# apple/ml-4m

Measured on AMD Instinct MI355X. Metric: multimodal tokens/sec (4M-B train step, whole job), higher is better.
Workload: dtype bf16; 1 GPU; 4M-B mod7 (fm_base_12e_12d_swiglu_nobias, 360.8M params, 8 input / 7 target modalities) masked-modeling train step, 224^2 token grids, 128 input + 128 target tokens/sample, AdamW; model=fm_base_12e_12d_swiglu_nobias, per_gpu_batch=256, global_batch=256, seq_len=256, parallelism=dp1

## Files before the change

include/fourm_hip.h:

```cpp
#ifndef FOURM_HIP_H
#define FOURM_HIP_H
#include <stdint.h>

#ifdef __cplusplus
extern "C" {
#endif

#define FM_ABI_VERSION 11
int fm_abi_version(void);
const char* fm_last_error(void);

enum fm_epilogue {
    FM_EPI_BF16 = 0,
    FM_EPI_GELU = 1,
    FM_EPI_RESIDUAL = 2,
    FM_EPI_SWIGLU = 3,
    FM_EPI_F32 = 4,
    FM_EPI_TANH = 5,
    FM_EPI_SWIGLU_BWD = 6,
    FM_EPI_GELU_BWD = 7,
    FM_EPI_QUICK_GELU = 8,
    FM_EPI_RELU = 9,
    FM_EPI_RELU_BWD = 10
};

typedef struct fm_gemm_group {
    const void* W;
    void* out;
    int32_t N, K, ldw, pad_;
} fm_gemm_group;

typedef struct fm_gemm_nt_args {
    const void* W; const void* W2; const void* X;
    void* out; void* out2; const void* res; const void* bias; const void* bias2;
    int32_t M, N, K, ldw, ldx, ldo, ldo2, ldr, Hp, epilogue;
    const fm_gemm_group* groups; const int32_t* tile_group; int32_t max_N;
    int32_t fixed_tiling;
    const int32_t* m_dev; const int32_t* row0_dev;
    void* splitk_ws; int64_t splitk_ws_bytes;
    int32_t conv_C, conv_H, conv_W, conv_Ho, conv_Wo, conv_stride, conv_up, conv_pad_;
} fm_gemm_nt_args;
int fm_gemm_nt(const fm_gemm_nt_args* args, void* stream);
void fm_set_gemm_nt_config(int cfg);
int fm_get_gemm_nt_config(void);
void fm_set_reserved_cus(int n);
int fm_get_reserved_cus(void);

typedef struct fm_gemm_tn_args {
    const void* A; const void* B; void* out;
    int32_t R, N, K, lda, ldb, ldo, a_cols, b_cols, splits, force_tr;
    const fm_gemm_group* groups; const int32_t* seg_start; const int32_t* seg_count;
    int32_t n_groups, max_N, max_R, pad_;
} fm_gemm_tn_args;
int fm_gemm_tn(const fm_gemm_tn_args* args, void* stream);
#define FM_TN_MAX_JOBS 16
typedef struct fm_gemm_tn_job {
    const void* A; const void* B; void* out;
    int32_t R, N, K, lda, ldb, ldo, a_cols, b_cols;
} fm_gemm_tn_job;
int fm_gemm_tn_multi(const fm_gemm_tn_job* jobs, int n_jobs, void* stream);
void fm_set_gemm_tn_config(int cfg);
int fm_get_gemm_tn_config(void);
void fm_set_tn_transpose_read(int on);
int fm_get_tn_transpose_read(void);

int fm_layernorm_fwd(const void* x, int ldx, const void* w, const void* b, void* y, int ldy, int y_is_f32,
                     void* mean, void* rstd, const int32_t* row_map, int R, int D, float eps, void* stream);
int fm_layernorm_fwd_res(const void* x, int ldx, const void* delta, int ldd, void* x_out, int ldxo, const void* w, const void* b,
                         void* y, int ldy, int y_is_f32, void* mean, void* rstd, const int32_t* row_map, int R, int D, float eps,
                         void* stream);
int fm_layernorm_bwd(const void* dy, int lddy, const int32_t* dy_row_map, const void* x, int ldx, const void* w,
                     const void* mean, const void* rstd, const void* dres, void* dx, int lddx, void* dx_bf16,
                     int lddxbf, void* dw, void* db, int R, int D, void* stream);
int fm_layernorm_bwd_h(const void* dy, int lddy, const void* h, int ldh, const void* x, int ldx, const void* w,
                       const void* mean, const void* rstd, const void* dres, void* dx, int lddx, void* dx_bf16,
                       int lddxbf, void* dw, int R, int D, void* stream);

int fm_headnorm_fwd(const void* x, int ldx, const void* w, const void* b, void* y, int ldy, void* stats, int R, int H, float eps,
                    void* stream);
int fm_headnorm_bwd(const void* dy, int lddy, const void* x, int ldx, const void* w, const void* stats, void* dx, int lddx, void* dw,
                    void* db, int R, int H, void* stream);

enum fm_mask_kind {
    FM_MASK_NONE = 0,
    FM_MASK_KEYPAD = 1,
    FM_MASK_DECODER = 2,
    FM_MASK_DENSE = 3
};
typedef struct fm_attn_args {
    const void* Q; const void* K; const void* V; void* O;
    void* stat_m; void* stat_l;
    int32_t ldq, ldk, ldv, ldo;
    int32_t B, H, Nq, Nk, head_dim, mask_kind;
    float scale; int32_t causal;
    const void* kpad; const int32_t* cs; const int16_t* modq; const int16_t* modk; const void* dense;
    const void* dO; void* dQ; void* dK; void* dV;
    int32_t lddo, lddq, lddk, lddv;
    int32_t force_tr;
    int32_t kv_batch_rows;
    int32_t zero_attn;
} fm_attn_args;
int fm_attn_fwd(const fm_attn_args* args, void* stream);
int fm_attn_bwd(const fm_attn_args* args, void* stream);
void fm_set_attn_transpose_read(int on);
int fm_get_attn_transpose_read(void);

#define FM_ATTN_DECODE_MAX_NK 8192
typedef struct fm_attn_decode_args {
    const void* q; void* k; const void* v; void* o;
    const void* q_w; const void* q_b; const void* k_w; const void* k_b;
    const void* kpad;
    int32_t ldq, ldk, ldv, ldo;
    int32_t B, H, Nk, kv_batch_rows, k_new_row, is_f32, zero_attn, pad_;
    float scale, eps;
} fm_attn_decode_args;
int fm_attn_decode(const fm_attn_decode_args* args, void* stream);

#define FM_MAX_MODS 24
enum fm_mod_kind {
    FM_KIND_TOK = 0,
    FM_KIND_PATCH = 1,
    FM_KIND_SEQ = 2,
    FM_KIND_SEQ_EMB = 3
};
typedef struct fm_mod_desc {
    const void* ids;
    const void* mask;
    const void* dam;
    const void* table;
    const void* pos;
    const void* mod_emb;
    const void* proj_bias;
    int32_t L;
    int32_t kind, ids_are_i64, mod_id;
    int32_t max_len;
    int32_t shifted;
    int32_t mask_stride, id_stride;
    int32_t patch, channels, grid_w, orig_dim;
    int32_t head_index;
    int32_t pad_;
} fm_mod_desc;

typedef struct fm_select_desc {
    fm_mod_desc mods[FM_MAX_MODS];
    int32_t n_mods, batch, dim, n_keep, n_reg, total_len, is_decoder;
    int32_t raw;
    const void* reg_tokens;
    const void* mask_token;
    void* tokens;
    void* emb;
    void* x0;
    void* out_mask;
    void* out_mod;
    void* slot_mod;
    void* slot_src;
    void* slot_pos;
    void* target_ids;
    void* out_cs;
    void* out_mod_pre;
    void* out_mod_index;
    void* patch_rows;
    void* seqemb_rows;
    int32_t patch_ld, seqemb_ld;
    int32_t rows_f32;
    int32_t pad2_;
} fm_select_desc;
int fm_select_embed(const fm_select_desc* desc, void* stream);

typedef struct fm_embed_bwd_mod {
    void* d_table;
    void* d_pos;
    void* d_mod_emb;
    void* d_proj_bias;
    int32_t kind, has_padding_idx, padding_idx, pad_;
} fm_embed_bwd_mod;
typedef struct fm_embed_bwd_desc {
    fm_embed_bwd_mod mods[FM_MAX_MODS];
    const void* dx;
    const void* slot_mod; const void* slot_src; const void* slot_pos;
    void* d_mask_token;
    void* d_reg_tokens;
    int32_t n_mods, batch, dim, Nt, lddx, is_decoder;
} fm_embed_bwd_desc;
int fm_embed_bwd(const fm_embed_bwd_desc* desc, void* stream);

int fm_dense_decoder_mask(const int32_t* cs, const int16_t* mod, void* out, int B, int M, int causal, int use_cs,
                          int use_sep, void* stream);

enum fm_loss_type { FM_LOSS_MOD = 0, FM_LOSS_TOKEN = 1 };
#define FM_SEG_ROWS 256
int fm_segment_rows(const int32_t* head_of_row, int R, int n_heads, int32_t* seg_start, int32_t* seg_count,
                    int32_t* perm, int32_t* row_to_padded, int32_t* tile_group, int Rp, void* stream);
int fm_gather_rows(const void* src, int ld_src, const int32_t* perm, void* dst, int ld_dst, int Rp, int D, void* stream);
int fm_cross_entropy(void* logits, int ldl, const int32_t* perm, const int32_t* tile_group, const int64_t* target_ids,
                     const int32_t* vocab, const int32_t* seg_start, const int32_t* seg_count, const void* grad_scale,
                     int loss_type, int n_heads, int Rp, int max_vocab, void* row_loss, void* row_lse, void* head_loss,
                     void* total_loss, int write_grad, void* stream);

int fm_swiglu_bwd(const void* da, int ldda, const void* gu, int ldgu, void* dgu, int lddgu, int R, int H, int Hp, void* stream);
int fm_gelu_bwd(const void* dh, int lddh, const void* pre, int ldp, void* dpre, int lddp, int R, int H, int Hp, void* stream);
typedef struct fm_shadow_desc {
    const void* src; void* dst;
    int32_t ld_src, ld_dst, rows, cols, transpose, tile_start;
    const void* col_scale;
    int32_t dst_f32, reserved;
} fm_shadow_desc;
int fm_shadow_refresh(const fm_shadow_desc* descs, int n_descs, int total_tiles, void* stream);
#define FM_FOLD_MAX_JOBS 48
typedef struct fm_fold_grad_job {
    const void* dWp; const void* W; const void* gamma; void* gW; void* ggamma;
    int32_t rows, cols, ld_dwp, reserved;
} fm_fold_grad_job;
int fm_fold_colscale_grad(const fm_fold_grad_job* jobs, int n_jobs, void* stream);

int fm_cast_pad(const void* src, int ld_src, void* dst, int ld_dst, int rows, int cols, void* stream);
int fm_transpose_cast_pad(const void* src, int ld_src, void* dst, int ld_dst, int dst_cols, int rows, int cols, void* stream);
int fm_colsum(const void* dy, int ldy, void* db, int R, int N, void* stream);
int fm_f32_to_bf16(const void* src, void* dst, int64_t n, void* stream);
int fm_bf16_to_f32_scaled(const void* src, void* dst, int64_t n, float scale, void* stream);
int fm_add_bf16_f32(const void* x, const void* delta, void* out, int64_t n, void* stream);
int fm_scale_rows_bf16(void* x, int ld, const void* scale, int rows_per_sample, int R, int N, void* stream);

int fm_vit_patch_rows(const void* pixels, void* rows, int ld, int B, int C, int H, int W, int P, int rows_f32, void* stream);
int fm_vit_emb_rows(const void* pos, const void* mod_emb, void* x, int ldx, int B, int Np, int D, void* stream);
int fm_vit_colsum(const void* dy, int ldy, void* db, int R, int N, void* ws, int64_t ws_bytes, void* stream);

int fm_clip_embed_ln(const void* patches, int ldp, int patches_f32, const void* cls, const void* pos, const void* w, const void* b,
                     void* out, int ldo, int B, int G, int D, float eps, void* stream);

// ... 179 lines not shown
```

ml-4m_amd/csrc/layernorm.hip:

```cpp
#include <algorithm>
#include "common.h"
#include "fourm_hip.h"

namespace {

constexpr int MAXC_LIMIT = 8;

__device__ __forceinline__ float4 ld4(const float* p, bool nt) {
    if (nt) { const f32x4_t t = __builtin_nontemporal_load((const f32x4_t*)p); return make_float4(t[0], t[1], t[2], t[3]); }
    return *(const float4*)p;
}
__device__ __forceinline__ uint2 ld2u(const bf16_t* p, bool nt) {
    typedef __attribute__((ext_vector_type(2))) unsigned int u2_t;
    if (nt) { const u2_t t = __builtin_nontemporal_load((const u2_t*)p); return make_uint2(t[0], t[1]); }
    return *(const uint2*)p;
}
template <typename T> __device__ __forceinline__ void store4(T* p, float a, float b, float c, float d);
template <> __device__ __forceinline__ void store4<float>(float* p, float a, float b, float c, float d) {
    *(float4*)p = make_float4(a, b, c, d);
}
template <> __device__ __forceinline__ void store4<bf16_t>(bf16_t* p, float a, float b, float c, float d) {
    *(uint2*)p = make_uint2(pack2bf(a, b), pack2bf(c, d));
}

template <typename OutT, int MAXC, bool RES = false>
__global__ __launch_bounds__(256) void ln_fwd_kernel(const float* __restrict__ x, int ldx, const float* __restrict__ w,
                                                     const float* __restrict__ b, OutT* __restrict__ y, int ldy,
                                                     float* __restrict__ mean, float* __restrict__ rstd,
                                                     const int* __restrict__ row_map, int R, int D, float eps,
                                                     const bf16_t* __restrict__ delta = nullptr, int ldd = 0, float* __restrict__ xo = nullptr, int ldxo = 0,
                                                     int nt_res = 0) {
    const int lane = threadIdx.x & 63, wave = threadIdx.x >> 6;
    const int nch = D >> 2;
    float4 ww[MAXC], bb[MAXC];
#pragma unroll
    for (int c = 0; c < MAXC; ++c) {
        const int ch = lane + 64 * c;
        ww[c] = ch < nch ? *(const float4*)(w + ch * 4) : make_float4(0.f, 0.f, 0.f, 0.f);
        bb[c] = (b && ch < nch) ? *(const float4*)(b + ch * 4) : make_float4(0.f, 0.f, 0.f, 0.f);
    }
    constexpr int NR = 2;
    for (int r0 = blockIdx.x * 4 + wave; r0 < R; r0 += gridDim.x * 4 * NR) {
        float4 v[NR][MAXC];
#pragma unroll
        for (int q = 0; q < NR; ++q) {
            const int r = r0 + q * gridDim.x * 4;
#pragma unroll
            for (int c = 0; c < MAXC; ++c) {
                const int ch = lane + 64 * c;
                v[q][c] = (ch < nch && r < R) ? ld4(x + (size_t)r * ldx + ch * 4, nt_res & 2) : make_float4(0.f, 0.f, 0.f, 0.f);
            }
        }
        if constexpr (RES) {
            uint2 dl[NR][MAXC];
#pragma unroll
            for (int q = 0; q < NR; ++q) {
                const int r = r0 + q * gridDim.x * 4;
#pragma unroll
                for (int c = 0; c < MAXC; ++c) {
                    const int ch = lane + 64 * c;
                    dl[q][c] = (ch < nch && r < R) ? ld2u(delta + (size_t)r * ldd + ch * 4, nt_res & 2) : make_uint2(0u, 0u);
                }
            }
#pragma unroll
            for (int q = 0; q < NR; ++q) {
                const int r = r0 + q * gridDim.x * 4;
#pragma unroll
                for (int c = 0; c < MAXC; ++c) {
                    const int ch = lane + 64 * c;
                    float d4[4];
                    unpack_bf4(dl[q][c], d4);
                    v[q][c].x += d4[0]; v[q][c].y += d4[1]; v[q][c].z += d4[2]; v[q][c].w += d4[3];
                    if (ch < nch && r < R) {
                        if (nt_res & 1) __builtin_nontemporal_store(f32x4_t{v[q][c].x, v[q][c].y, v[q][c].z, v[q][c].w}, (f32x4_t*)(xo + (size_t)r * ldxo + ch * 4));
                        else *(float4*)(xo + (size_t)r * ldxo + ch * 4) = v[q][c];
                    }
                }
            }
        }
#pragma unroll
        for (int q = 0; q < NR; ++q) {
            const int r = r0 + q * gridDim.x * 4;
            if (r >= R) continue;
            float s = 0.f;
#pragma unroll
            for (int c = 0; c < MAXC; ++c) s += (v[q][c].x + v[q][c].y) + (v[q][c].z + v[q][c].w);
            const float mu = wave_sum(s) / (float)D;
            float sq = 0.f;
#pragma unroll
            for (int c = 0; c < MAXC; ++c) {
                const int ch = lane + 64 * c;
                if (ch < nch) {
                    const float a0 = v[q][c].x - mu, a1 = v[q][c].y - mu, a2 = v[q][c].z - mu, a3 = v[q][c].w - mu;
                    sq += (a0 * a0 + a1 * a1) + (a2 * a2 + a3 * a3);
                }
            }
            const float rs = rsqrtf(wave_sum(sq) / (float)D + eps);
            if (lane == 0) {
                if (mean) mean[r] = mu;
                if (rstd) rstd[r] = rs;
            }
            const int dst = row_map ? row_map[r] : r;
            if (dst < 0) continue;
            OutT* yr = y + (size_t)dst * ldy;
#pragma unroll
            for (int c = 0; c < MAXC; ++c) {
                const int ch = lane + 64 * c;
                if (ch < nch)
                    store4<OutT>(yr + ch * 4, (v[q][c].x - mu) * rs * ww[c].x + bb[c].x, (v[q][c].y - mu) * rs * ww[c].y + bb[c].y,
                                 (v[q][c].z - mu) * rs * ww[c].z + bb[c].z, (v[q][c].w - mu) * rs * ww[c].w + bb[c].w);
            }
        }
    }
}

static int ln_nt_flags() {
    static const int f = [] { const char* e = getenv("FOURM_LN_NT"); return e ? atoi(e) : 24; }();
    return f;
}
static int bwd_rows(int R) {
    static const int env = [] { const char* e = getenv("FOURM_LN_BWD_ROWS"); return e ? atoi(e) : 0; }();
    if (env >= 4) return env;
    return R >= 512 * 64 ? 64 : 32;
}

template <int MAXC, bool FROM_H = false, bool HAS_DB = true>
__global__ __launch_bounds__(256) void ln_bwd_kernel(const bf16_t* __restrict__ dy, int lddy, const int* __restrict__ dy_row_map,
                                                     const bf16_t* __restrict__ h, int ldh,
                                                     const float* __restrict__ x, int ldx, const float* __restrict__ w,
                                                     const float* __restrict__ mean, const float* __restrict__ rstd,
                                                     const float* dres, float* dx, int lddx, bf16_t* __restrict__ dx_bf, int lddxbf,
                                                     float* __restrict__ dw, float* __restrict__ db, int R, int D, int BWD_ROWS, int nt_dx) {
    extern __shared__ __attribute__((aligned(16))) char smem[];
    float* red = (float*)smem;
    const int lane = threadIdx.x & 63, wave = threadIdx.x >> 6;
    const int nch = D >> 2;
    float4 aw[MAXC], ab[MAXC], wv[MAXC], iw[FROM_H ? MAXC : 1];
    bool from_x[FROM_H ? MAXC : 1];
#pragma unroll
    for (int c = 0; c < MAXC; ++c) {
        aw[c] = ab[c] = make_float4(0.f, 0.f, 0.f, 0.f);
        const int ch = lane + 64 * c;
        wv[c] = ch < nch ? *(const float4*)(w + ch * 4) : make_float4(0.f, 0.f, 0.f, 0.f);
        if constexpr (FROM_H) {
            from_x[c] = fminf(fminf(fabsf(wv[c].x), fabsf(wv[c].y)), fminf(fabsf(wv[c].z), fabsf(wv[c].w))) < 1e-20f;
            iw[c] = from_x[c] ? make_float4(0.f, 0.f, 0.f, 0.f) : make_float4(1.f / wv[c].x, 1.f / wv[c].y, 1.f / wv[c].z, 1.f / wv[c].w);
        }
    }
    const int r_end = min(R, (int)(blockIdx.x + 1) * BWD_ROWS);
    constexpr int NR = 2;
    for (int r0 = blockIdx.x * BWD_ROWS + wave; r0 < r_end; r0 += 4 * NR) {
        uint2 dyp[NR][MAXC], hp[NR][FROM_H ? MAXC : 1];
        float4 xv[NR][MAXC], rv[NR][MAXC];
        float mu[NR], rs[NR];
        bool live[NR];
#pragma unroll
        for (int q = 0; q < NR; ++q) {
            const int r = r0 + 4 * q;
            live[q] = r < r_end;
            const int rr = live[q] ? r : r0;
            const int src = dy_row_map ? dy_row_map[rr] : rr;
            mu[q] = mean[rr]; rs[q] = rstd[rr];
#pragma unroll
            for (int c = 0; c < MAXC; ++c) {
                const int ch = lane + 64 * c;
                dyp[q][c] = make_uint2(0u, 0u);
                xv[q][c] = rv[q][c] = make_float4(0.f, 0.f, 0.f, 0.f);
                if (ch < nch && live[q]) {
                    if (src >= 0) dyp[q][c] = ld2u(dy + (size_t)src * lddy + ch * 4, nt_dx & 2);
                    if constexpr (FROM_H) {
                        hp[q][c] = ld2u(h + (size_t)rr * ldh + ch * 4, nt_dx & 4);
                        if (from_x[c]) xv[q][c] = *(const float4*)(x + (size_t)rr * ldx + ch * 4);
                    } else xv[q][c] = *(const float4*)(x + (size_t)rr * ldx + ch * 4);
                    if (dres) rv[q][c] = ld4(dres + (size_t)rr * lddx + ch * 4, nt_dx & 2);
                }
            }
        }
#pragma unroll
        for (int q = 0; q < NR; ++q) {
            if (!live[q]) continue;
            const int r = r0 + 4 * q;
            float4 g[MAXC], xh[MAXC];
            float s1 = 0.f, s2 = 0.f;
#pragma unroll
            for (int c = 0; c < MAXC; ++c) {
                const int ch = lane + 64 * c;
                g[c] = xh[c] = make_float4(0.f, 0.f, 0.f, 0.f);
                if (ch < nch) {
                    const uint2 p = dyp[q][c];
                    const float4 d = make_float4(bf2f((bf16_t)(p.x & 0xffff)), bf2f((bf16_t)(p.x >> 16)), bf2f((bf16_t)(p.y & 0xffff)), bf2f((bf16_t)(p.y >> 16)));
                    const float4 v = xv[q][c];
                    xh[c] = make_float4((v.x - mu[q]) * rs[q], (v.y - mu[q]) * rs[q], (v.z - mu[q]) * rs[q], (v.w - mu[q]) * rs[q]);
                    if constexpr (FROM_H) {
                        const uint2 hh = hp[q][c];
                        if (!from_x[c]) xh[c] = make_float4(bf2f((bf16_t)(hh.x & 0xffff)) * iw[c].x, bf2f((bf16_t)(hh.x >> 16)) * iw[c].y,
                                                            bf2f((bf16_t)(hh.y & 0xffff)) * iw[c].z, bf2f((bf16_t)(hh.y >> 16)) * iw[c].w);
                    }
                    aw[c].x += d.x * xh[c].x; aw[c].y += d.y * xh[c].y; aw[c].z += d.z * xh[c].z; aw[c].w += d.w * xh[c].w;
                    if constexpr (HAS_DB) { ab[c].x += d.x; ab[c].y += d.y; ab[c].z += d.z; ab[c].w += d.w; }
                    g[c] = make_float4(d.x * wv[c].x, d.y * wv[c].y, d.z * wv[c].z, d.w * wv[c].w);
                    s1 += (g[c].x + g[c].y) + (g[c].z + g[c].w);
                    s2 += (g[c].x * xh[c].x + g[c].y * xh[c].y) + (g[c].z * xh[c].z + g[c].w * xh[c].w);
                }
            }
            const float m1 = wave_sum(s1) / (float)D, m2 = wave_sum(s2) / (float)D;
#pragma unroll
            for (int c = 0; c < MAXC; ++c) {
                const int ch = lane + 64 * c;
                if (ch < nch) {
                    const float4 t = rv[q][c];
                    const float4 o = make_float4(rs[q] * (g[c].x - m1 - xh[c].x * m2) + t.x, rs[q] * (g[c].y - m1 - xh[c].y * m2) + t.y,
                                                 rs[q] * (g[c].z - m1 - xh[c].z * m2) + t.z, rs[q] * (g[c].w - m1 - xh[c].w * m2) + t.w);
                    if (nt_dx & 1) __builtin_nontemporal_store(f32x4_t{o.x, o.y, o.z, o.w}, (f32x4_t*)(dx + (size_t)r * lddx + ch * 4));
                    else *(float4*)(dx + (size_t)r * lddx + ch * 4) = o;
                    if (dx_bf) *(uint2*)(dx_bf + (size_t)r * lddxbf + ch * 4) = make_uint2(pack2bf(o.x, o.y), pack2bf(o.z, o.w));
                }
            }
        }
    }
    if (!dw && !db) return;
#pragma unroll
    for (int c = 0; c < MAXC; ++c) {
        const int ch = lane + 64 * c;
        if (ch < nch) {
            *(float4*)(red + (size_t)wave * D + ch * 4) = aw[c];
            if constexpr (HAS_DB) *(float4*)(red + (size_t)(4 + wave) * D + ch * 4) = ab[c];
        }
    }
    __syncthreads();
    for (int i = threadIdx.x; i < D; i += 256) {
        if (dw) unsafeAtomicAdd(dw + i, (red[i] + red[D + i]) + (red[2 * D + i] + red[3 * D + i]));
        if constexpr (HAS_DB) if (db) unsafeAtomicAdd(db + i, (red[4 * D + i] + red[5 * D + i]) + (red[6 * D + i] + red[7 * D + i]));
    }
}


__device__ __forceinline__ float group16_sum(float v) {
    v += __shfl_xor(v, 1, 64); v += __shfl_xor(v, 2, 64); v += __shfl_xor(v, 4, 64); v += __shfl_xor(v, 8, 64);
    return v;
}

__global__ __launch_bounds__(256) void headnorm_fwd_kernel(const bf16_t* __restrict__ x, int ldx, const float* __restrict__ w,
                                                           const float* __restrict__ b, bf16_t* __restrict__ y, int ldy,
                                                           float2* __restrict__ stats, int R, int H, float eps) {
    const int sub = threadIdx.x & 15;
    const float4 wv = *(const float4*)(w + sub * 4);
    const float4 bv = b ? *(const float4*)(b + sub * 4) : make_float4(0.f, 0.f, 0.f, 0.f);
    const size_t total = (size_t)R * H;
    for (size_t v = (size_t)blockIdx.x * 16 + (threadIdx.x >> 4); v < total; v += (size_t)gridDim.x * 16) {
        const int r = v / H, h = v % H;
        const uint2 p = *(const uint2*)(x + (size_t)r * ldx + h * 64 + sub * 4);
        const float e[4] = {bf2f((bf16_t)(p.x & 0xffff)), bf2f((bf16_t)(p.x >> 16)), bf2f((bf16_t)(p.y & 0xffff)), bf2f((bf16_t)(p.y >> 16))};
        const float mean = group16_sum(e[0] + e[1] + e[2] + e[3]) * (1.0f / 64.0f);
        float q = 0.f;
#pragma unroll
        for (int i = 0; i < 4; ++i) q += (e[i] - mean) * (e[i] - mean);
        const float rs = rsqrtf(group16_sum(q) * (1.0f / 64.0f) + eps);
        const float o0 = (e[0] - mean) * rs * wv.x + bv.x, o1 = (e[1] - mean) * rs * wv.y + bv.y;
        const float o2 = (e[2] - mean) * rs * wv.z + bv.z, o3 = (e[3] - mean) * rs * wv.w + bv.w;
        *(uint2*)(y + (size_t)r * ldy + h * 64 + sub * 4) = make_uint2(pack2bf(o0, o1), pack2bf(o2, o3));
        if (sub == 0 && stats) stats[v] = make_float2(mean, rs);
    }
}

__global__ __launch_bounds__(256) void headnorm_bwd_kernel(const bf16_t* __restrict__ dy, int lddy, const bf16_t* __restrict__ x, int ldx,
                                                           const float* __restrict__ w, const float2* __restrict__ stats,
                                                           bf16_t* __restrict__ dx, int lddx, float* __restrict__ dw, float* __restrict__ db,
                                                           int R, int H) {
    __shared__ float red[2][16][64];
    const int sub = threadIdx.x & 15, grp = threadIdx.x >> 4;
    const float4 wv = *(const float4*)(w + sub * 4);
    const float wj[4] = {wv.x, wv.y, wv.z, wv.w};
    float aw[4] = {0.f, 0.f, 0.f, 0.f}, ab[4] = {0.f, 0.f, 0.f, 0.f};
    const size_t total = (size_t)R * H;
    for (size_t v = (size_t)blockIdx.x * 16 + grp; v < total; v += (size_t)gridDim.x * 16) {
        const int r = v / H, h = v % H;
        const uint2 px = *(const uint2*)(x + (size_t)r * ldx + h * 64 + sub * 4);
        const uint2 pd = *(const uint2*)(dy + (size_t)r * lddy + h * 64 + sub * 4);
        const float2 st = stats[v];
        const float e[4] = {bf2f((bf16_t)(px.x & 0xffff)), bf2f((bf16_t)(px.x >> 16)), bf2f((bf16_t)(px.y & 0xffff)), bf2f((bf16_t)(px.y >> 16))};
        const float d[4] = {bf2f((bf16_t)(pd.x & 0xffff)), bf2f((bf16_t)(pd.x >> 16)), bf2f((bf16_t)(pd.y & 0xffff)), bf2f((bf16_t)(pd.y >> 16))};
        float xh[4], g[4], s1 = 0.f, s2 = 0.f;
#pragma unroll
        for (int i = 0; i < 4; ++i) {
            xh[i] = (e[i] - st.x) * st.y;
            g[i] = d[i] * wj[i];
            s1 += g[i]; s2 += g[i] * xh[i];
            aw[i] += d[i] * xh[i]; ab[i] += d[i];
        }
        s1 = group16_sum(s1) * (1.0f / 64.0f); s2 = group16_sum(s2) * (1.0f / 64.0f);
        float o[4];
#pragma unroll
        for (int i = 0; i < 4; ++i) o[i] = st.y * (g[i] - s1 - xh[i] * s2);
        *(uint2*)(dx + (size_t)r * lddx + h * 64 + sub * 4) = make_uint2(pack2bf(o[0], o[1]), pack2bf(o[2], o[3]));
    }
#pragma unroll
    for (int i = 0; i < 4; ++i) { red[0][grp][sub * 4 + i] = aw[i]; red[1][grp][sub * 4 + i] = ab[i]; }
    __syncthreads();
    if (threadIdx.x < 128) {
        const int which = threadIdx.x >> 6, c = threadIdx.x & 63;
        float s = 0.f;
#pragma unroll
        for (int gq = 0; gq < 16; ++gq) s += red[which][gq][c];
        float* dst = which ? db : dw;
        if (dst) unsafeAtomicAdd(dst + c, s);
    }
}

}

static int chunks_for(int D) { const int c = (D / 4 + 63) / 64; return c <= 2 ? 2 : c <= 3 ? 3 : c <= 4 ? 4 : 8; }

extern "C" int fm_layernorm_fwd(const void* x, int ldx, const void* w, const void* b, void* y, int ldy, int y_is_f32,
                                void* mean, void* rstd, const int32_t* row_map, int R, int D, float eps, void* stream) {
    FM_CHECK_ARG(x && w && y, "fm_layernorm_fwd: null pointer");
    FM_CHECK_ARG(R > 0 && D > 0 && D % 4 == 0 && D <= 64 * 4 * MAXC_LIMIT, "fm_layernorm_fwd: D=%d must be a multiple of 4 and <= %d", D, 64 * 4 * MAXC_LIMIT);
    FM_CHECK_ARG(ldx % 4 == 0 && ldy % 4 == 0, "fm_layernorm_fwd: leading dims must be multiples of 4");
    int grid = (R + 3) / 4;
    if (grid > 256 * 16) grid = 256 * 16;
#define LN_FWD(T, C)                                                                                                        \
    hipLaunchKernelGGL((ln_fwd_kernel<T, C>), dim3(grid), dim3(256), 0, (hipStream_t)stream, (const float*)x, ldx, (const float*)w, \
                       (const float*)b, (T*)y, ldy, (float*)mean, (float*)rstd, row_map, R, D, eps)
#define LN_FWD_C(T)                                    \
    switch (chunks_for(D)) {                           \
        case 2: LN_FWD(T, 2); break;                   \
        case 3: LN_FWD(T, 3); break;                   \
        case 4: LN_FWD(T, 4); break;                   \
        default: LN_FWD(T, 8); break;                  \
    }
    if (y_is_f32) { LN_FWD_C(float) } else { LN_FWD_C(bf16_t) }
#undef LN_FWD_C
#undef LN_FWD
    FM_CHECK_LAUNCH("fm_layernorm_fwd");
    return 0;
}

extern "C" int fm_layernorm_fwd_res(const void* x, int ldx, const void* delta, int ldd, void* x_out, int ldxo, const void* w, const void* b,
                                    void* y, int ldy, int y_is_f32, void* mean, void* rstd, const int32_t* row_map, int R, int D, float eps,
                                    void* stream) {
    FM_CHECK_ARG(x && delta && x_out && w && y, "fm_layernorm_fwd_res: null pointer");
    FM_CHECK_ARG(R > 0 && D > 0 && D % 4 == 0 && D <= 64 * 4 * MAXC_LIMIT, "fm_layernorm_fwd_res: D=%d must be a multiple of 4 and <= %d", D, 64 * 4 * MAXC_LIMIT);
    FM_CHECK_ARG(ldx % 4 == 0 && ldy % 4 == 0 && ldd % 4 == 0 && ldxo % 4 == 0, "fm_layernorm_fwd_res: leading dims must be multiples of 4");
    FM_CHECK_ARG((((uintptr_t)delta) & 7) == 0 && (((uintptr_t)x_out | (uintptr_t)x) & 15) == 0, "fm_layernorm_fwd_res: alignment (delta 8 B, x / x_out 16 B)");
    int grid = (R + 3) / 4;
    if (grid > 256 * 16) grid = 256 * 16;
#define LN_FWD(T, C)                                                                                                        \
    hipLaunchKernelGGL((ln_fwd_kernel<T, C, true>), dim3(grid), dim3(256), 0, (hipStream_t)stream, (const float*)x, ldx, (const float*)w, \
                       (const float*)b, (T*)y, ldy, (float*)mean, (float*)rstd, row_map, R, D, eps, (const bf16_t*)delta, ldd, (float*)x_out, ldxo, (ln_nt_flags() & 1) | ((ln_nt_flags() >> 1) & 2))
#define LN_FWD_C(T)                                    \
    switch (chunks_for(D)) {                           \
        case 2: LN_FWD(T, 2); break;                   \
        case 3: LN_FWD(T, 3); break;                   \
        case 4: LN_FWD(T, 4); break;                   \
        default: LN_FWD(T, 8); break;                  \
    }
    if (y_is_f32) { LN_FWD_C(float) } else { LN_FWD_C(bf16_t) }
#undef LN_FWD_C
#undef LN_FWD
    FM_CHECK_LAUNCH("fm_layernorm_fwd_res");
    return 0;
}

static int layernorm_bwd_launch(const void* dy, int lddy, const int32_t* dy_row_map, const void* h, int ldh, const void* x, int ldx, const void* w,
                                const void* mean, const void* rstd, const void* dres, void* dx, int lddx, void* dx_bf16,
                                int lddxbf, void* dw, void* db, int R, int D, void* stream) {
    FM_CHECK_ARG(dy && x && w && mean && rstd && dx, "fm_layernorm_bwd: null pointer");
    FM_CHECK_ARG(!h || ldh % 4 == 0, "fm_layernorm_bwd_h: ldh must be a multiple of 4");
    FM_CHECK_ARG(R > 0 && D > 0 && D % 4 == 0 && D <= 64 * 4 * MAXC_LIMIT, "fm_layernorm_bwd: D=%d unsupported", D);
    FM_CHECK_ARG(ldx % 4 == 0 && lddy % 4 == 0 && lddx % 4 == 0 && lddxbf % 4 == 0, "fm_layernorm_bwd: leading dims must be multiples of 4");
    const int BWD_ROWS = bwd_rows(R);
    const int grid = (R + BWD_ROWS - 1) / BWD_ROWS;
    const size_t lds = (size_t)8 * D * sizeof(float);
#define LN_BWD_(C, FH)                                                                                                      \
    {                                                                                                                       \
        auto k = ln_bwd_kernel<C, FH, !FH>;                                                                                     \
        static bool once = (hipFuncSetAttribute((const void*)k, hipFuncAttributeMaxDynamicSharedMemorySize, 8 * 2048 * 4) == hipSuccess); \
        (void)once;                                                                                                         \
        hipLaunchKernelGGL(k, dim3(grid), dim3(256), lds, (hipStream_t)stream, (const bf16_t*)dy, lddy, dy_row_map, (const bf16_t*)h, ldh, \
                           (const float*)x, ldx, (const float*)w, (const float*)mean, (const float*)rstd, (const float*)dres, (float*)dx, lddx, \
                           (bf16_t*)dx_bf16, lddxbf, (float*)dw, (float*)db, R, D, BWD_ROWS, ((ln_nt_flags() >> 1) & 1) | ((ln_nt_flags() >> 2) & 2) | ((ln_nt_flags() >> 2) & 4));                               \
    }
#define LN_BWD(C) { if (h) LN_BWD_(C, true) else LN_BWD_(C, false) }
    switch (chunks_for(D)) {
        case 2: LN_BWD(2) break;
        case 3: LN_BWD(3) break;
        case 4: LN_BWD(4) break;
        default: LN_BWD(8) break;
    }
#undef LN_BWD
#undef LN_BWD_
    FM_CHECK_LAUNCH("fm_layernorm_bwd");
    return 0;
}

extern "C" int fm_layernorm_bwd(const void* dy, int lddy, const int32_t* dy_row_map, const void* x, int ldx, const void* w,
                                const void* mean, const void* rstd, const void* dres, void* dx, int lddx, void* dx_bf16,
                                int lddxbf, void* dw, void* db, int R, int D, void* stream) {
    return layernorm_bwd_launch(dy, lddy, dy_row_map, nullptr, 0, x, ldx, w, mean, rstd, dres, dx, lddx, dx_bf16, lddxbf, dw, db, R, D, stream);
}

extern "C" int fm_layernorm_bwd_h(const void* dy, int lddy, const void* h, int ldh, const void* x, int ldx, const void* w,
                                  const void* mean, const void* rstd, const void* dres, void* dx, int lddx, void* dx_bf16,
                                  int lddxbf, void* dw, int R, int D, void* stream) {
    FM_CHECK_ARG(h, "fm_layernorm_bwd_h: null pointer");
    return layernorm_bwd_launch(dy, lddy, nullptr, h, ldh, x, ldx, w, mean, rstd, dres, dx, lddx, dx_bf16, lddxbf, dw, nullptr, R, D, stream);
}

extern "C" int fm_headnorm_fwd(const void* x, int ldx, const void* w, const void* b, void* y, int ldy, void* stats, int R, int H, float eps,
                               void* stream) {
    FM_CHECK_ARG(x && w && y && R > 0 && H > 0, "fm_headnorm_fwd: bad argument");
    FM_CHECK_ARG(ldx % 4 == 0 && ldy % 4 == 0 && ((((uintptr_t)x | (uintptr_t)y) & 7) == 0) && ((((uintptr_t)w | (uintptr_t)b) & 15) == 0),
                 "fm_headnorm_fwd: alignment (x/y 8 B, w/b 16 B, leading dims %% 4)");
    const size_t total = (size_t)R * H;
    const int grid = (int)std::min<size_t>((total + 15) / 16, 256 * 32);
    hipLaunchKernelGGL(headnorm_fwd_kernel, dim3(grid), dim3(256), 0, (hipStream_t)stream, (const bf16_t*)x, ldx, (const float*)w, (const float*)b,
                       (bf16_t*)y, ldy, (float2*)stats, R, H, eps);
    FM_CHECK_LAUNCH("fm_headnorm_fwd");
    return 0;
}

extern "C" int fm_headnorm_bwd(const void* dy, int lddy, const void* x, int ldx, const void* w, const void* stats, void* dx, int lddx, void* dw,
                               void* db, int R, int H, void* stream) {
    FM_CHECK_ARG(dy && x && w && stats && dx && R > 0 && H > 0, "fm_headnorm_bwd: bad argument");
    FM_CHECK_ARG(ldx % 4 == 0 && lddy % 4 == 0 && lddx % 4 == 0 && ((((uintptr_t)x | (uintptr_t)dy | (uintptr_t)dx) & 7) == 0) &&
                     ((((uintptr_t)w) & 15) == 0), "fm_headnorm_bwd: alignment (x/dy/dx 8 B, w 16 B, leading dims %% 4)");
    const size_t total = (size_t)R * H;
    const int grid = (int)std::min<size_t>((total + 15) / 16, 256 * 8);
    hipLaunchKernelGGL(headnorm_bwd_kernel, dim3(grid), dim3(256), 0, (hipStream_t)stream, (const bf16_t*)dy, lddy, (const bf16_t*)x, ldx,
                       (const float*)w, (const float2*)stats, (bf16_t*)dx, lddx, (float*)dw, (float*)db, R, H);
    FM_CHECK_LAUNCH("fm_headnorm_bwd");
    return 0;
}
```

ml-4m_amd/csrc/select_embed.hip:

```cpp
#include "common.h"
#include "fourm_hip.h"

namespace {

constexpr int MAXPOS = 8192;
constexpr int MAXKEEP = 1024;

struct SelArgs {
    fm_select_desc d;
};

__device__ __forceinline__ long long load_id(const void* ids, int is64, size_t i) {
    return is64 ? ((const long long*)ids)[i] : (long long)((const int*)ids)[i];
}

__device__ __forceinline__ int block_scan_excl(int v, int* wave_tot , int* total) {
    const int lane = threadIdx.x & 63, wave = threadIdx.x >> 6;
    const int inc = wave_scan_incl(v);
    if (lane == 63) wave_tot[wave] = inc;
    __syncthreads();
    int base = 0, tot = 0;
#pragma unroll
    for (int w = 0; w < 4; ++w) {
        const int t = wave_tot[w];
// ... 70 lines not shown
                const int s = base + lane;
                int v = 0;
                if (s < d.n_keep) {
                    const int p = slot_p[s];
                    const int m = mod_of(p);
                    const fm_mod_desc& md = d.mods[m];
                    v = ((const int*)md.dam)[(size_t)b * md.mask_stride + (p - mod_off[m])];
                }
                const int inc = wave_scan_incl(v);
                if (s < d.n_keep) cs_scan[s] = run + inc;
                run += __shfl(inc, 63, 64);
            }
        }
        __syncthreads();
    }

    const int D = d.dim, nch = D >> 2;
    const int Nt = d.n_reg + d.n_keep;
    for (int s = wave + 4 * blockIdx.y; s < Nt; s += 4 * gridDim.y) {
        const size_t orow = (size_t)b * Nt + s;
        float* tok_o = (float*)d.tokens + orow * D;
        float* emb_o = (float*)d.emb + orow * D;
        float* x0_o = d.x0 ? (float*)d.x0 + orow * D : nullptr;
        if (s < d.n_reg) {
            for (int c = lane; c < nch; c += 64) {
                const float4 t = *(const float4*)((const float*)d.reg_tokens + (size_t)s * D + c * 4);
                *(float4*)(tok_o + c * 4) = t;
                *(float4*)(emb_o + c * 4) = make_float4(0.f, 0.f, 0.f, 0.f);
                if (x0_o) *(float4*)(x0_o + c * 4) = t;
            }
            if (lane == 0) {
                ((uint8_t*)d.out_mask)[orow] = 0;
                ((int16_t*)d.out_mod)[orow] = -1;
                ((int32_t*)d.slot_mod)[orow] = -2;
                ((int32_t*)d.slot_src)[orow] = s;
                ((int32_t*)d.slot_pos)[orow] = 0;
            }
            const int esz = d.rows_f32 ? 2 : 1;
            if (d.patch_rows) {
                uint2* pr = (uint2*)((char*)d.patch_rows + orow * d.patch_ld * (size_t)(2 * esz));
                for (int f = lane; f < d.patch_ld / 4 * esz; f += 64) pr[f] = make_uint2(0u, 0u);
            }
            if (d.seqemb_rows) {
                uint2* sr = (uint2*)((char*)d.seqemb_rows + orow * d.seqemb_ld * (size_t)(2 * esz));
                for (int f = lane; f < d.seqemb_ld / 4 * esz; f += 64) sr[f] = make_uint2(0u, 0u);
            }
            continue;
        }
        const int sk = s - d.n_reg;
        const int p = slot_p[sk];
        const int m = mod_of(p);
        const fm_mod_desc& md = d.mods[m];
        const int j = p - mod_off[m];
        const bool masked = (flag[p] & 1) == 0;
        const bool own_unmasked = (flag[p] & 2) != 0;
        const bool raw = d.raw != 0;
        long long id = 0;
        int posrow = 0;
        if (md.kind == FM_KIND_TOK || md.kind == FM_KIND_SEQ) id = load_id(md.ids, md.ids_are_i64, (size_t)b * md.id_stride + j);
        if (md.kind == FM_KIND_SEQ || md.kind == FM_KIND_SEQ_EMB) {
            posrow = rank_pos[p] - rank_pos[mod_off[m]];
            if (d.is_decoder && posrow >= md.max_len) posrow = 0;
        } else {
            posrow = j;
        }
        if (lane == 0) {
            ((uint8_t*)d.out_mask)[orow] = masked ? 1 : 0;
            ((int16_t*)d.out_mod)[orow] = (masked && !raw) ? (int16_t)-1 : (int16_t)md.mod_id;
            ((int32_t*)d.slot_mod)[orow] = (masked && !raw) ? -1 : m;
            ((int32_t*)d.slot_src)[orow] = (md.kind == FM_KIND_TOK || md.kind == FM_KIND_SEQ) ? (int)id : j;
            ((int32_t*)d.slot_pos)[orow] = posrow;
            if (d.is_decoder) {
                long long tgt = md.shifted ? load_id(md.ids, md.ids_are_i64, (size_t)b * md.id_stride + j + 1) : id;
                ((long long*)d.target_ids)[orow] = (masked && !raw) ? 0 : tgt;
                ((int32_t*)d.out_cs)[orow] = raw ? 0 : cs_scan[sk];
                ((int16_t*)d.out_mod_pre)[orow] = (int16_t)md.mod_id;
                ((int32_t*)d.out_mod_index)[orow] = masked ? -1 : md.head_index;
            }
        }
        const float* trow = nullptr;
        if (!masked || raw) {
            if (d.is_decoder && md.kind == FM_KIND_TOK && d.raw != 2) trow = (const float*)d.mask_token;
            else if (md.kind == FM_KIND_TOK || md.kind == FM_KIND_SEQ) trow = (const float*)md.table + (size_t)id * D;
            else if (md.kind == FM_KIND_SEQ_EMB) trow = (const float*)md.proj_bias;
        }
        const float* prow = (const float*)md.pos + (size_t)posrow * D;
        const float* mrow = (const float*)md.mod_emb;
        const bool seq_kind = md.kind == FM_KIND_SEQ || md.kind == FM_KIND_SEQ_EMB;
        const bool with_emb = raw ? true : !masked;
        const bool with_pos = raw ? (!seq_kind || own_unmasked) : true;
        for (int c = lane; c < nch; c += 64) {
            float4 t = make_float4(0.f, 0.f, 0.f, 0.f), e = make_float4(0.f, 0.f, 0.f, 0.f);
            if (trow) t = *(const float4*)(trow + c * 4);
            if (with_emb) {
                const float4 mm = *(const float4*)(mrow + c * 4);
                float4 pp = make_float4(0.f, 0.f, 0.f, 0.f);
                if (with_pos) pp = *(const float4*)(prow + c * 4);
                e = make_float4(pp.x + mm.x, pp.y + mm.y, pp.z + mm.z, pp.w + mm.w);
            }
            *(float4*)(tok_o + c * 4) = t;
            *(float4*)(emb_o + c * 4) = e;
            if (x0_o) *(float4*)(x0_o + c * 4) = make_float4(t.x + e.x, t.y + e.y, t.z + e.z, t.w + e.w);
        }
        if (d.patch_rows && d.rows_f32) {
            float* pr = (float*)d.patch_rows + orow * d.patch_ld;
            const bool here = (!masked || raw) && md.kind == FM_KIND_PATCH;
            const int ps = md.patch, C = md.channels, gw = md.grid_w;
            const float* img = (const float*)md.ids + (size_t)b * md.id_stride;
            for (int f = lane; f < d.patch_ld; f += 64) {
                float v = 0.f;
                if (here && f < ps * ps * C) {
                    const int gy = j / gw, gx = j % gw, Wd = gw * ps, Hd = (md.L / gw) * ps;
                    const int c = f % C, px = (f / C) % ps, py = f / (C * ps);
                    v = img[((size_t)c * Hd + gy * ps + py) * Wd + gx * ps + px];
                }
                pr[f] = v;
            }
        } else if (d.patch_rows) {
            bf16_t* pr = (bf16_t*)d.patch_rows + orow * d.patch_ld;
            if ((!masked || raw) && md.kind == FM_KIND_PATCH) {
                const int ps = md.patch, C = md.channels, gw = md.grid_w;
                const int gy = j / gw, gx = j % gw;
                const float* img = (const float*)md.ids + (size_t)b * md.id_stride;
                const int Wd = gw * ps, Hd = (md.L / gw) * ps;
                for (int f = lane; f < d.patch_ld; f += 64) {
                    float v = 0.f;
                    if (f < ps * ps * C) {
                        const int c = f % C, px = (f / C) % ps, py = f / (C * ps);
                        v = img[((size_t)c * Hd + gy * ps + py) * Wd + gx * ps + px];
                    }
                    pr[f] = f2bf(v);
                }
            } else {
                for (int f = lane; f < d.patch_ld / 4; f += 64) *(uint2*)(pr + f * 4) = make_uint2(0u, 0u);
            }
        }
        if (d.seqemb_rows && d.rows_f32) {
            float* sr = (float*)d.seqemb_rows + orow * d.seqemb_ld;
            const bool here = (!masked || raw) && md.kind == FM_KIND_SEQ_EMB;
            const float* src = (const float*)md.ids + (size_t)b * md.id_stride + (size_t)j * md.orig_dim;
            for (int f = lane; f < d.seqemb_ld; f += 64) sr[f] = (here && f < md.orig_dim) ? src[f] : 0.f;
        } else if (d.seqemb_rows) {
            bf16_t* sr = (bf16_t*)d.seqemb_rows + orow * d.seqemb_ld;
            if ((!masked || raw) && md.kind == FM_KIND_SEQ_EMB) {
                const float* src = (const float*)md.ids + (size_t)b * md.id_stride + (size_t)j * md.orig_dim;
                for (int f = lane; f < d.seqemb_ld; f += 64) sr[f] = f2bf(f < md.orig_dim ? src[f] : 0.f);
            } else {
                for (int f = lane; f < d.seqemb_ld / 4; f += 64) *(uint2*)(sr + f * 4) = make_uint2(0u, 0u);
            }
        }
    }
}

__global__ __launch_bounds__(256) void embed_bwd_kernel(fm_embed_bwd_desc d) {
    extern __shared__ __attribute__((aligned(16))) char smem[];
    float* acc = (float*)smem;
    const int D = d.dim, nch = D >> 2;
    const int b = blockIdx.x, lane = threadIdx.x & 63, wave = threadIdx.x >> 6;
    const int rows = d.n_mods + 1;
    for (int i = threadIdx.x; i < rows * D; i += 256) acc[i] = 0.f;
    __shared__ int used[FM_MAX_MODS + 1];
    if (threadIdx.x <= FM_MAX_MODS) used[threadIdx.x] = 0;
    __syncthreads();
    constexpr int MAXQ = 8;
    const int parts = 4 * gridDim.y, part = wave + 4 * blockIdx.y;
    const int per = (d.Nt + parts - 1) / parts, s_lo = part * per, s_hi = min(d.Nt, s_lo + per);
    float4 racc[MAXQ];
    int cur = -1;
    bool cur_mask = false;
    auto flush = [&]() {
        if (cur < 0) return;
#pragma unroll
        for (int q = 0; q < MAXQ; ++q) {
            const int c = lane + 64 * q;
            if (c >= nch) break;
            float* a0 = acc + (size_t)cur * D + c * 4;
            atomicAdd(a0, racc[q].x); atomicAdd(a0 + 1, racc[q].y); atomicAdd(a0 + 2, racc[q].z); atomicAdd(a0 + 3, racc[q].w);
            if (cur_mask) {
                float* a1 = acc + (size_t)d.n_mods * D + c * 4;
                atomicAdd(a1, racc[q].x); atomicAdd(a1 + 1, racc[q].y); atomicAdd(a1 + 2, racc[q].z); atomicAdd(a1 + 3, racc[q].w);
            }
        }
    };
    for (int s = s_lo; s < s_hi; ++s) {
        const size_t row = (size_t)b * d.Nt + s;
        const int m = ((const int32_t*)d.slot_mod)[row];
        if (m == -1) continue;
        const float* g = (const float*)d.dx + row * d.lddx;
        if (m == -2) {
            if (d.d_reg_tokens)
                for (int c = lane; c < D; c += 64) unsafeAtomicAdd((float*)d.d_reg_tokens + (size_t)s * D + c, g[c]);
            continue;
        }
        const fm_embed_bwd_mod& md = d.mods[m];
        const int src = ((const int32_t*)d.slot_src)[row];
        const int posrow = ((const int32_t*)d.slot_pos)[row];
        const bool to_mask_token = d.is_decoder && md.kind == FM_KIND_TOK;
        if (m != cur) {
            flush();
            cur = m; cur_mask = to_mask_token;
#pragma unroll
            for (int q = 0; q < MAXQ; ++q) racc[q] = make_float4(0.f, 0.f, 0.f, 0.f);
            if (lane == 0) { used[m] = 1; if (to_mask_token) used[d.n_mods] = 1; }
        }
        float* trow = nullptr;
        if (to_mask_token) {}
        else if ((md.kind == FM_KIND_TOK || md.kind == FM_KIND_SEQ) && md.d_table && !(md.has_padding_idx && src == md.padding_idx))
            trow = (float*)md.d_table + (size_t)src * D;
        else if (md.kind == FM_KIND_SEQ_EMB && md.d_proj_bias) trow = (float*)md.d_proj_bias;
        float* prow = md.d_pos ? (float*)md.d_pos + (size_t)posrow * D : nullptr;
#pragma unroll
        for (int q = 0; q < MAXQ; ++q) {
            const int c = lane + 64 * q;
            if (c >= nch) break;
            const float4 v = *(const float4*)(g + c * 4);
            racc[q].x += v.x; racc[q].y += v.y; racc[q].z += v.z; racc[q].w += v.w;
            if (trow) {
                unsafeAtomicAdd(trow + c * 4, v.x); unsafeAtomicAdd(trow + c * 4 + 1, v.y);
                unsafeAtomicAdd(trow + c * 4 + 2, v.z); unsafeAtomicAdd(trow + c * 4 + 3, v.w);
            }
            if (prow) {
                unsafeAtomicAdd(prow + c * 4, v.x); unsafeAtomicAdd(prow + c * 4 + 1, v.y);
                unsafeAtomicAdd(prow + c * 4 + 2, v.z); unsafeAtomicAdd(prow + c * 4 + 3, v.w);
            }
        }
    }
    flush();
    __syncthreads();
    for (int m = 0; m < d.n_mods; ++m) {
        if (!used[m] || !d.mods[m].d_mod_emb) continue;
        for (int c = threadIdx.x; c < D; c += 256) unsafeAtomicAdd((float*)d.mods[m].d_mod_emb + c, acc[(size_t)m * D + c]);
    }
    if (used[d.n_mods] && d.d_mask_token)
        for (int c = threadIdx.x; c < D; c += 256) unsafeAtomicAdd((float*)d.d_mask_token + c, acc[(size_t)d.n_mods * D + c]);
}

__global__ void dense_decoder_mask_kernel(const int32_t* cs, const int16_t* mod, uint8_t* out, int B, int M, int causal, int use_cs, int use_sep) {
    const size_t i = (size_t)blockIdx.x * 256 + threadIdx.x;
    if (i >= (size_t)B * M * M) return;
    const int k = i % M, q = (i / M) % M, b = i / ((size_t)M * M);
    bool blk = false;
    if (causal) blk = k > q;
    else if (use_cs) blk = k >= cs[(size_t)b * M + q];
    if (use_sep) blk = blk || (mod[(size_t)b * M + q] != mod[(size_t)b * M + k]);
    out[i] = blk ? 1 : 0;
}

}

extern "C" int fm_select_embed(const fm_select_desc* d, void* stream) {
    FM_CHECK_ARG(d && d->tokens && d->emb && d->out_mask && d->out_mod && d->slot_mod && d->slot_src && d->slot_pos, "fm_select_embed: null output");
    FM_CHECK_ARG(d->n_mods > 0 && d->n_mods <= FM_MAX_MODS, "fm_select_embed: n_mods=%d out of range (max %d)", d->n_mods, FM_MAX_MODS);
    FM_CHECK_ARG(d->dim > 0 && d->dim % 4 == 0, "fm_select_embed: dim must be a multiple of 4");
    FM_CHECK_ARG(d->batch > 0 && d->n_keep > 0 && d->n_keep <= (d->raw ? MAXPOS : MAXKEEP), "fm_select_embed: n_keep=%d out of range (max %d)", d->n_keep,
                 d->raw ? MAXPOS : MAXKEEP);
    int total = 0;
    for (int m = 0; m < d->n_mods; ++m) {
        const fm_mod_desc& md = d->mods[m];
        FM_CHECK_ARG(md.L > 0 && md.mask && md.pos && md.mod_emb, "fm_select_embed: modality %d incomplete", m);
        FM_CHECK_ARG(md.kind != FM_KIND_PATCH || (d->patch_rows && md.ids), "fm_select_embed: pixel modality needs patch_rows and pixels");
        FM_CHECK_ARG(md.kind != FM_KIND_SEQ_EMB || (d->seqemb_rows && md.ids), "fm_select_embed: seq_emb modality needs seqemb_rows");
        FM_CHECK_ARG(!((md.kind == FM_KIND_TOK || md.kind == FM_KIND_SEQ) && !(d->is_decoder && md.kind == FM_KIND_TOK)) || md.table, "fm_select_embed: modality %d needs a table", m);
        FM_CHECK_ARG(!d->is_decoder || md.dam || d->raw, "fm_select_embed: decoder modality %d needs decoder_attention_mask", m);
        FM_CHECK_ARG(!(d->raw == 2 && md.kind == FM_KIND_TOK) || md.table, "fm_select_embed: modality %d needs a table", m);
        total += md.L;
    }
    FM_CHECK_ARG(total == d->total_len, "fm_select_embed: total_len=%d but the modalities sum to %d", d->total_len, total);
    FM_CHECK_ARG(total <= MAXPOS, "fm_select_embed: %d concatenated positions exceed %d", total, MAXPOS);
    FM_CHECK_ARG(d->n_keep <= total, "fm_select_embed: n_keep=%d exceeds the %d available positions", d->n_keep, total);
    FM_CHECK_ARG(d->raw >= 0 && d->raw <= 2 && (!d->raw || (d->n_keep == total && d->n_reg == 0)),
                 "fm_select_embed: raw views cover every position (n_keep == total_len) and carry no register tokens");
    FM_CHECK_ARG(!d->is_decoder || (d->target_ids && d->out_cs && d->out_mod_pre && d->out_mod_index && d->mask_token), "fm_select_embed: decoder outputs missing");
    FM_CHECK_ARG(d->n_reg == 0 || d->reg_tokens, "fm_select_embed: register tokens missing");
    FM_CHECK_ARG(d->patch_ld % 4 == 0 && d->seqemb_ld % 4 == 0, "fm_select_embed: side buffers need ld %% 4 == 0");
    const size_t lds = (size_t)total * 9 + (size_t)d->n_keep * 4 + 16;
    static bool once = (hipFuncSetAttribute((const void*)select_embed_kernel, hipFuncAttributeMaxDynamicSharedMemorySize, MAXPOS * 9 + MAXPOS * 4 + 16) == hipSuccess);
    (void)once;
    SelArgs A; A.d = *d;
    const int slices = d->batch >= 2048 ? 1 : d->batch >= 1024 ? 2 : 4;
    hipLaunchKernelGGL(select_embed_kernel, dim3(d->batch, slices), dim3(256), lds, (hipStream_t)stream, A);
    FM_CHECK_LAUNCH("fm_select_embed");
    return 0;
}

extern "C" int fm_embed_bwd(const fm_embed_bwd_desc* d, void* stream) {
    FM_CHECK_ARG(d && d->dx && d->slot_mod && d->slot_src && d->slot_pos, "fm_embed_bwd: null pointer");
    FM_CHECK_ARG(d->n_mods > 0 && d->n_mods <= FM_MAX_MODS && d->dim % 4 == 0 && d->dim <= 2048 && d->lddx % 4 == 0, "fm_embed_bwd: bad shape (dim <= 2048)");
    const size_t lds = (size_t)(d->n_mods + 1) * d->dim * sizeof(float);
    FM_CHECK_ARG(lds <= 150 * 1024, "fm_embed_bwd: %zu bytes of LDS needed", lds);
    static bool once = (hipFuncSetAttribute((const void*)embed_bwd_kernel, hipFuncAttributeMaxDynamicSharedMemorySize, 150 * 1024) == hipSuccess);
    (void)once;
    const int slices = d->batch >= 2048 ? 1 : d->batch >= 1024 ? 2 : 4;
    hipLaunchKernelGGL(embed_bwd_kernel, dim3(d->batch, slices), dim3(256), lds, (hipStream_t)stream, *d);
    FM_CHECK_LAUNCH("fm_embed_bwd");
    return 0;
}

extern "C" int fm_dense_decoder_mask(const int32_t* cs, const int16_t* mod, void* out, int B, int M, int causal, int use_cs, int use_sep, void* stream) {
    FM_CHECK_ARG(out && (causal || !use_cs || cs) && (!use_sep || mod), "fm_dense_decoder_mask: null pointer");
    const size_t n = (size_t)B * M * M;
    hipLaunchKernelGGL(dense_decoder_mask_kernel, dim3((n + 255) / 256), dim3(256), 0, (hipStream_t)stream, cs, mod, (uint8_t*)out, B, M, causal, use_cs, use_sep);
    FM_CHECK_LAUNCH("fm_dense_decoder_mask");
    return 0;
}
```

ml-4m_amd/fourm/hip/_lib.py:

```python
import ctypes as C
import os

FM_MAX_MODS = 24
_LIB_PATH = os.environ.get("FOURM_HIP_LIB") or os.path.join(os.path.dirname(os.path.dirname(os.path.abspath(__file__))), "_lib", "libfourm_hip.so")


class FourmHipUnavailable(ImportError):
    pass


def _load():
    if not os.path.exists(_LIB_PATH):
        raise FourmHipUnavailable(
            f"{_LIB_PATH} is missing - build the gfx950 kernels first: python ml-4m_amd/build_ext.py "
            "(the 4M hot path has no fallback implementation)")
    return C.CDLL(_LIB_PATH)


lib = _load()
lib.fm_last_error.restype = C.c_char_p
lib.fm_abi_version.restype = C.c_int
ABI_VERSION = 11
if lib.fm_abi_version() != ABI_VERSION:
    raise FourmHipUnavailable(f"libfourm_hip.so ABI {lib.fm_abi_version()} != expected {ABI_VERSION}; rebuild")

vp, i32, i64, f32 = C.c_void_p, C.c_int32, C.c_int64, C.c_float

EPI_BF16, EPI_GELU, EPI_RESIDUAL, EPI_SWIGLU, EPI_F32, EPI_TANH, EPI_SWIGLU_BWD, EPI_GELU_BWD, EPI_QUICK_GELU = 0, 1, 2, 3, 4, 5, 6, 7, 8
EPI_RELU, EPI_RELU_BWD = 9, 10
MASK_NONE, MASK_KEYPAD, MASK_DECODER, MASK_DENSE = 0, 1, 2, 3
KIND_TOK, KIND_PATCH, KIND_SEQ, KIND_SEQ_EMB = 0, 1, 2, 3
LOSS_MOD, LOSS_TOKEN = 0, 1


class GemmGroup(C.Structure):
    _fields_ = [("W", vp), ("out", vp), ("N", i32), ("K", i32), ("ldw", i32), ("pad_", i32)]


class GemmNTArgs(C.Structure):
    _fields_ = [("W", vp), ("W2", vp), ("X", vp), ("out", vp), ("out2", vp), ("res", vp), ("bias", vp), ("bias2", vp),
                ("M", i32), ("N", i32), ("K", i32), ("ldw", i32), ("ldx", i32), ("ldo", i32), ("ldo2", i32), ("ldr", i32),
                ("Hp", i32), ("epilogue", i32), ("groups", vp), ("tile_group", vp), ("max_N", i32), ("fixed_tiling", i32),
                ("m_dev", vp), ("row0_dev", vp), ("splitk_ws", vp), ("splitk_ws_bytes", i64),
                ("conv_C", i32), ("conv_H", i32), ("conv_W", i32), ("conv_Ho", i32), ("conv_Wo", i32), ("conv_stride", i32), ("conv_up", i32), ("conv_pad_", i32)]


class GemmTNArgs(C.Structure):
    _fields_ = [("A", vp), ("B", vp), ("out", vp), ("R", i32), ("N", i32), ("K", i32), ("lda", i32), ("ldb", i32),
                ("ldo", i32), ("a_cols", i32), ("b_cols", i32), ("splits", i32), ("force_tr", i32), ("groups", vp),
                ("seg_start", vp), ("seg_count", vp), ("n_groups", i32), ("max_N", i32), ("max_R", i32), ("pad_", i32)]


class GemmTNJob(C.Structure):
    _fields_ = [("A", vp), ("B", vp), ("out", vp), ("R", i32), ("N", i32), ("K", i32), ("lda", i32), ("ldb", i32),
                ("ldo", i32), ("a_cols", i32), ("b_cols", i32)]


TN_MAX_JOBS = 16


class AttnArgs(C.Structure):
    _fields_ = [("Q", vp), ("K", vp), ("V", vp), ("O", vp), ("stat_m", vp), ("stat_l", vp),
                ("ldq", i32), ("ldk", i32), ("ldv", i32), ("ldo", i32),
                ("B", i32), ("H", i32), ("Nq", i32), ("Nk", i32), ("head_dim", i32), ("mask_kind", i32),
                ("scale", f32), ("causal", i32),
                ("kpad", vp), ("cs", vp), ("modq", vp), ("modk", vp), ("dense", vp),
                ("dO", vp), ("dQ", vp), ("dK", vp), ("dV", vp),
                ("lddo", i32), ("lddq", i32), ("lddk", i32), ("lddv", i32), ("force_tr", i32), ("kv_batch_rows", i32), ("zero_attn", i32)]


class AttnDecodeArgs(C.Structure):
    _fields_ = [("q", vp), ("k", vp), ("v", vp), ("o", vp), ("q_w", vp), ("q_b", vp), ("k_w", vp), ("k_b", vp), ("kpad", vp),
                ("ldq", i32), ("ldk", i32), ("ldv", i32), ("ldo", i32),
                ("B", i32), ("H", i32), ("Nk", i32), ("kv_batch_rows", i32), ("k_new_row", i32), ("is_f32", i32), ("zero_attn", i32), ("pad_", i32),
                ("scale", f32), ("eps", f32)]


class ModDesc(C.Structure):
    _fields_ = [("ids", vp), ("mask", vp), ("dam", vp), ("table", vp), ("pos", vp), ("mod_emb", vp), ("proj_bias", vp),
                ("L", i32), ("kind", i32), ("ids_are_i64", i32), ("mod_id", i32), ("max_len", i32), ("shifted", i32),
                ("mask_stride", i32), ("id_stride", i32), ("patch", i32), ("channels", i32), ("grid_w", i32),
                ("orig_dim", i32), ("head_index", i32), ("pad_", i32)]


class ShadowDesc(C.Structure):
    _fields_ = [("src", vp), ("dst", vp), ("ld_src", i32), ("ld_dst", i32), ("rows", i32), ("cols", i32),
                ("transpose", i32), ("tile_start", i32), ("col_scale", vp), ("dst_f32", i32), ("reserved", i32)]


FOLD_MAX_JOBS = 48


class FoldGradJob(C.Structure):
    _fields_ = [("dWp", vp), ("W", vp), ("gamma", vp), ("gW", vp), ("ggamma", vp), ("rows", i32), ("cols", i32), ("ld_dwp", i32), ("reserved", i32)]


class GemmF32Args(C.Structure):
    _fields_ = [("X", vp), ("W", vp), ("W2", vp), ("out", vp), ("out2", vp), ("res", vp), ("bias", vp), ("bias2", vp),
                ("sxm", i64), ("sxk", i64), ("swn", i64), ("swk", i64),
                ("M", i32), ("N", i32), ("K", i32), ("ldo", i32), ("ldo2", i32), ("ldr", i32), ("Hp", i32), ("epilogue", i32),
                ("accumulate", i32), ("max_N", i32), ("seg_rows", i32), ("n_groups", i32),
                ("groups", vp), ("tile_group", vp), ("seg_start", vp), ("seg_count", vp)]


class SpanMaskArgs(C.Structure):
    _fields_ = [("ids", vp), ("len", vp), ("unit", vp), ("noise", vp), ("keep_prob", vp), ("r_choice", vp), ("input_budget", vp), ("target_budget", vp),
                ("sentinel_ids", vp), ("emb", vp), ("emb_out", vp), ("src", vp), ("tensor", vp), ("input_mask", vp), ("target_mask", vp),
                ("decoder_attention_mask", vp), ("tries", vp),
                ("B", i32), ("ld_ids", i32), ("T", i32), ("ld_noise", i32), ("n_sentinels", i32), ("max_tokens", i32), ("vocab_offset", i32), ("pad_id", i32),
                ("emb_rows", i32), ("emb_dim", i32)]


class AdamWJob(C.Structure):
    _fields_ = [("p", vp), ("g", vp), ("m", vp), ("v", vp), ("dst_plain", vp), ("dst_t", vp),
                ("rows", i32), ("cols", i32), ("ld_plain", i32), ("ld_t", i32), ("tile_start", i32), ("pad_", i32)]


class SelectDesc(C.Structure):
    _fields_ = [("mods", ModDesc * FM_MAX_MODS),
                ("n_mods", i32), ("batch", i32), ("dim", i32), ("n_keep", i32), ("n_reg", i32), ("total_len", i32),
                ("is_decoder", i32), ("raw", i32),
                ("reg_tokens", vp), ("mask_token", vp),
                ("tokens", vp), ("emb", vp), ("x0", vp), ("out_mask", vp), ("out_mod", vp), ("slot_mod", vp),
                ("slot_src", vp), ("slot_pos", vp), ("target_ids", vp), ("out_cs", vp), ("out_mod_pre", vp),
                ("out_mod_index", vp), ("patch_rows", vp), ("seqemb_rows", vp), ("patch_ld", i32), ("seqemb_ld", i32),
                ("rows_f32", i32), ("pad2_", i32)]


class EmbedBwdMod(C.Structure):
    _fields_ = [("d_table", vp), ("d_pos", vp), ("d_mod_emb", vp), ("d_proj_bias", vp),
                ("kind", i32), ("has_padding_idx", i32), ("padding_idx", i32), ("pad_", i32)]


class EmbedBwdDesc(C.Structure):
    _fields_ = [("mods", EmbedBwdMod * FM_MAX_MODS), ("dx", vp), ("slot_mod", vp), ("slot_src", vp), ("slot_pos", vp),
                ("d_mask_token", vp), ("d_reg_tokens", vp),
                ("n_mods", i32), ("batch", i32), ("dim", i32), ("Nt", i32), ("lddx", i32), ("is_decoder", i32)]


class EmaJob(C.Structure):
    _fields_ = [("ema", vp), ("model", vp), ("n", i64), ("first_chunk", i64)]


def _sig(name, *argtypes):
    fn = getattr(lib, name)
    fn.argtypes = list(argtypes)
    fn.restype = C.c_int
    return fn


P = C.POINTER
gemm_nt = _sig("fm_gemm_nt", P(GemmNTArgs), vp)
gemm_tn = _sig("fm_gemm_tn", P(GemmTNArgs), vp)
gemm_tn_multi = _sig("fm_gemm_tn_multi", P(GemmTNJob), C.c_int, vp)
layernorm_fwd = _sig("fm_layernorm_fwd", vp, i32, vp, vp, vp, i32, i32, vp, vp, vp, i32, i32, f32, vp)
layernorm_fwd_res = _sig("fm_layernorm_fwd_res", vp, i32, vp, i32, vp, i32, vp, vp, vp, i32, i32, vp, vp, vp, i32, i32, f32, vp)
layernorm_bwd = _sig("fm_layernorm_bwd", vp, i32, vp, vp, i32, vp, vp, vp, vp, vp, i32, vp, i32, vp, vp, i32, i32, vp)
layernorm_bwd_h = _sig("fm_layernorm_bwd_h", vp, i32, vp, i32, vp, i32, vp, vp, vp, vp, vp, i32, vp, i32, vp, i32, i32, vp)
attn_fwd = _sig("fm_attn_fwd", P(AttnArgs), vp)
attn_bwd = _sig("fm_attn_bwd", P(AttnArgs), vp)
attn_decode = _sig("fm_attn_decode", P(AttnDecodeArgs), vp)
ATTN_DECODE_MAX_NK = 8192
select_embed = _sig("fm_select_embed", P(SelectDesc), vp)
embed_bwd = _sig("fm_embed_bwd", P(EmbedBwdDesc), vp)
dense_decoder_mask = _sig("fm_dense_decoder_mask", vp, vp, vp, i32, i32, i32, i32, i32, vp)
segment_rows = _sig("fm_segment_rows", vp, i32, i32, vp, vp, vp, vp, vp, i32, vp)
gather_rows = _sig("fm_gather_rows", vp, i32, vp, vp, i32, i32, i32, vp)
cross_entropy = _sig("fm_cross_entropy", vp, i32, vp, vp, vp, vp, vp, vp, vp, i32, i32, i32, i32, vp, vp, vp, vp, i32, vp)
swiglu_bwd = _sig("fm_swiglu_bwd", vp, i32, vp, i32, vp, i32, i32, i32, i32, vp)
gelu_bwd = _sig("fm_gelu_bwd", vp, i32, vp, i32, vp, i32, i32, i32, i32, vp)
cast_pad = _sig("fm_cast_pad", vp, i32, vp, i32, i32, i32, vp)
transpose_cast_pad = _sig("fm_transpose_cast_pad", vp, i32, vp, i32, i32, i32, i32, vp)
colsum = _sig("fm_colsum", vp, i32, vp, i32, i32, vp)
shadow_refresh = _sig("fm_shadow_refresh", vp, i32, i32, vp)
fold_colscale_grad = _sig("fm_fold_colscale_grad", vp, i32, vp)
headnorm_fwd = _sig("fm_headnorm_fwd", vp, i32, vp, vp, vp, i32, vp, i32, i32, C.c_float, vp)
headnorm_bwd = _sig("fm_headnorm_bwd", vp, i32, vp, i32, vp, vp, vp, i32, vp, vp, i32, i32, vp)
f32_to_bf16 = _sig("fm_f32_to_bf16", vp, vp, i64, vp)
bf16_to_f32_scaled = _sig("fm_bf16_to_f32_scaled", vp, vp, i64, f32, vp)
add_bf16_f32 = _sig("fm_add_bf16_f32", vp, vp, vp, i64, vp)
lib.fm_set_reserved_cus.argtypes = [C.c_int]
lib.fm_get_reserved_cus.restype = C.c_int
lib.fm_get_reserved_cus.argtypes = []
adamw = _sig("fm_adamw", vp, vp, vp, vp, i64, f32, f32, f32, f32, f32, i64, vp, vp, vp, vp)
adamw_shadow = _sig("fm_adamw_shadow", vp, i32, i32, f32, f32, f32, f32, f32, i64, vp, vp, vp, vp)
sumsq = _sig("fm_sumsq", vp, i64, vp, vp)
clip_coef = _sig("fm_clip_coef", vp, f32, vp, vp, vp)
sample_tokens = _sig("fm_sample_tokens", vp, i32, i32, i32, i32, f32, i32, f32, vp, vp, vp, vp)
maskgit_commit = _sig("fm_maskgit_commit", vp, vp, vp, i32, i32, i32, vp, i32, i32, vp, vp, vp, vp)
gemm_f32 = _sig("fm_gemm_f32", P(GemmF32Args), vp)
attn_f32_fwd = _sig("fm_attn_f32_fwd", P(AttnArgs), vp)
attn_f32_bwd = _sig("fm_attn_f32_bwd", P(AttnArgs), vp)
layernorm_bwd_f32 = _sig("fm_layernorm_bwd_f32", vp, i32, vp, vp, i32, vp, vp, vp, vp, vp, i32, vp, i32, vp, vp, i32, i32, vp)
headnorm_f32_fwd = _sig("fm_headnorm_f32_fwd", vp, i32, vp, vp, vp, i32, vp, i32, i32, C.c_float, vp)
headnorm_f32_bwd = _sig("fm_headnorm_f32_bwd", vp, i32, vp, i32, vp, vp, vp, i32, vp, vp, i32, i32, vp)
swiglu_bwd_f32 = _sig("fm_swiglu_bwd_f32", vp, i32, vp, i32, vp, i32, i32, i32, i32, vp)
gelu_bwd_f32 = _sig("fm_gelu_bwd_f32", vp, i32, vp, i32, vp, i32, i32, i32, vp)
colsum_f32 = _sig("fm_colsum_f32", vp, i32, vp, i32, i32, vp)
cross_entropy_f32 = _sig("fm_cross_entropy_f32", vp, i32, vp, vp, vp, vp, vp, vp, vp, i32, i32, i32, i32, vp, vp, vp, vp, i32, vp)
vq_patchify = _sig("fm_vq_patchify", vp, vp, i32, i32, i32, i32, i32, i32, vp)
l2norm_rows = _sig("fm_l2norm_rows", vp, i32, vp, i32, i32, i32, vp)
vq_assign = _sig("fm_vq_assign", vp, i32, vp, vp, i32, i32, i32, i32, i32, vp, vp, i32, vp, vp, vp)
lib.fm_set_tn_transpose_read.argtypes = [C.c_int]
lib.fm_set_gemm_tn_config.argtypes = [C.c_int]
lib.fm_set_attn_transpose_read.argtypes = [C.c_int]

lib.fm_set_gemm_nt_config.argtypes = [C.c_int]
lib.fm_lab_set.argtypes = [C.c_int, C.c_int]
lib.fm_lab_set.restype = None
vq_code_stats = _sig("fm_vq_code_stats", vp, i32, vp, i32, i32, i32, vp, vp, vp)
vq_ema_update = _sig("fm_vq_ema_update", vp, vp, vp, vp, i32, i32, f32, vp)
vq_code_bias = _sig("fm_vq_code_bias", vp, i32, i32, vp, vp)
vq_assign_bias = _sig("fm_vq_assign_bias", vp, i32, vp, vp, vp, i32, i32, i32, i32, i32, vp, vp, i32, vp, vp, vp)
vq_code_stats_raw = _sig("fm_vq_code_stats_raw", vp, i32, vp, i32, i32, i32, vp, vp, vp)
vq_ema_update_euclid = _sig("fm_vq_ema_update_euclid", vp, vp, vp, vp, vp, vp, i32, i32, f32, f32, vp)
vq_unpatchify = _sig("fm_vq_unpatchify", vp, i32, vp, i32, i32, i32, i32, i32, vp)
VQ_WIDE_TILE, CONVNEXT_MAX_C = 128, 4
vq_assign_wide = _sig("fm_vq_assign_wide", vp, i32, vp, vp, i32, i32, i32, i32, vp, vp, i32, vp, vp, vp)
memcodes_assign = _sig("fm_memcodes_assign", vp, i32, vp, vp, i32, i32, i32, i32, i32, vp, vp, i32, vp, vp, vp)
convnext_block = _sig("fm_convnext_block", vp, vp, vp, vp, vp, vp, vp, vp, vp, vp, vp, i32, i32, i32, i32, f32, vp)
vq_latent_grad = _sig("fm_vq_latent_grad", vp, i32, vp, vp, vp, i32, vp, f32, vp, i32, vp, i32, i32, vp)
tanh_bwd_f32 = _sig("fm_tanh_bwd_f32", vp, vp, vp, i32, i32, i32, vp)
embed_rows_f32 = _sig("fm_embed_rows_f32", vp, vp, vp, i32, i32, i32, vp)
vq_patchify_ex = _sig("fm_vq_patchify_ex", vp, vp, vp, vp, vp, vp, i32, i32, i32, i32, i32, i32, vp)
vq_cls_emb_bwd = _sig("fm_vq_cls_emb_bwd", vp, i32, vp, vp, i32, i32, i32, i32, i32, vp)
vq_latent_grad_normalized = _sig("fm_vq_latent_grad_normalized", vp, i32, vp, vp, vp, i32, vp, f32, vp, i32, vp, i32, i32, vp)
scale_rows_bf16 = _sig("fm_scale_rows_bf16", vp, i32, vp, i32, i32, i32, vp)
image_mask = _sig("fm_image_mask", vp, vp, vp, i32, i32, vp, vp, vp, vp)
token_budgets = _sig("fm_token_budgets", vp, vp, vp, vp, vp, vp, vp, i32, i32, i32, i32, vp, vp, vp)
span_mask = _sig("fm_span_mask", P(SpanMaskArgs), vp)
guidance_combine = _sig("fm_guidance_combine", vp, i32, i32, vp, i32, i32, f32, vp, i32, i32, i32, i32, vp)
unpack_image_u8 = _sig("fm_unpack_image_u8", vp, vp, i32, i32, i32, i32, P(C.c_float), P(C.c_float), vp)
unpack_ids_u16 = _sig("fm_unpack_ids_u16", vp, vp, i64, vp)
unpack_mask_bits = _sig("fm_unpack_mask_bits", vp, vp, i32, i32, vp)
decoder_attention_from_target = _sig("fm_decoder_attention_from_target", vp, vp, i32, i32, vp)
split3_bf16 = _sig("fm_split3_bf16", vp, i32, vp, i32, i32, i32, i32, i32, vp)
unet_im2col = _sig("fm_unet_im2col", vp, i32, i32, vp, i32, i32, i32, i32, vp, i32, i32, i32, i32, i32, i32, i32, i32, vp)
groupnorm_nhwc = _sig("fm_groupnorm_nhwc", vp, i32, vp, i32, vp, vp, vp, i32, vp, i32, i32, i32, i32, f32, i32, vp)
add_bf16 = _sig("fm_add_bf16", vp, i32, vp, i32, vp, i32, i64, i32, vp)
silu_f32_to_bf16 = _sig("fm_silu_f32_to_bf16", vp, vp, i64, vp)
timestep_embedding = _sig("fm_timestep_embedding", vp, vp, i32, i32, i32, f32, vp)
unet_attention = _sig("fm_unet_attention", vp, i32, vp, i32, i32, i32, i32, i32, vp)
unet_im2col_f32 = _sig("fm_unet_im2col_f32", vp, i32, i32, vp, i32, i32, i32, i32, vp, i32, i32, i32, i32, i32, i32, i32, i32, vp)
groupnorm_nhwc_f32 = _sig("fm_groupnorm_nhwc_f32", vp, i32, vp, i32, vp, vp, vp, i32, i32, i32, i32, i32, f32, i32, vp)
unet_attention_f32 = _sig("fm_unet_attention_f32", vp, i32, vp, i32, i32, i32, i32, i32, vp)
add_f32 = _sig("fm_add_f32", vp, i32, vp, i32, vp, i32, i64, i32, vp)
silu_f32 = _sig("fm_silu_f32", vp, vp, i64, vp)
timestep_embedding_f32 = _sig("fm_timestep_embedding_f32", vp, vp, i32, i32, i32, f32, vp)
unet_col2im_f32 = _sig("fm_unet_col2im_f32", vp, i32, vp, i32, i32, i32, i32, i32, i32, i32, i32, i32, vp)
groupnorm_nhwc_bwd_f32 = _sig("fm_groupnorm_nhwc_bwd_f32", vp, i32, vp, i32, vp, i32, vp, vp, vp, i32, vp, vp, vp, i32, vp, i32, i32, i32, i32, f32, i32, vp)
unet_attention_bwd_f32 = _sig("fm_unet_attention_bwd_f32", vp, i32, vp, i32, vp, i32, vp, i32, i32, i32, i32, vp)
silu_bwd_f32 = _sig("fm_silu_bwd_f32", vp, vp, vp, i64, vp)
diffusion_x0 = _sig("fm_diffusion_x0", vp, vp, f32, f32, vp, i64, vp)
quantile_abs = _sig("fm_quantile_abs", vp, i32, i64, f32, vp, vp)
diffusion_step = _sig("fm_diffusion_step", vp, vp, f32, f32, vp, vp, vp, f32, f32, f32, f32, vp, vp, i32, i64, vp)
lora_apply = _sig("fm_lora_apply", vp, i32, vp, i64, i64, vp, i64, i64, vp, i32, f32, vp, i32, i32, i32, i32, i32, i32, vp)
lora_grad = _sig("fm_lora_grad", vp, i32, vp, vp, i64, i64, f32, i32, i32, i32, i32, i32, vp)
vit_patch_rows = _sig("fm_vit_patch_rows", vp, vp, i32, i32, i32, i32, i32, i32, i32, vp)
vit_emb_rows = _sig("fm_vit_emb_rows", vp, vp, vp, i32, i32, i32, i32, vp)
vit_colsum = _sig("fm_vit_colsum", vp, i32, vp, i32, i32, vp, i64, vp)
clip_embed_ln = _sig("fm_clip_embed_ln", vp, i32, i32, vp, vp, vp, vp, vp, i32, i32, i32, i32, f32, vp)
FEAT_COSINE, FEAT_L1 = 0, 1
feat_distance = _sig("fm_feat_distance", vp, i32, vp, i32, i32, i32, i32, i32, vp, vp, i32, vp)
quick_gelu_bwd = _sig("fm_quick_gelu_bwd", vp, i32, vp, i32, vp, i32, i32, i32, i32, vp)
quick_gelu_bwd_f32 = _sig("fm_quick_gelu_bwd_f32", vp, i32, vp, i32, vp, i32, i32, i32, vp)
clip_embed_ln_bwd = _sig("fm_clip_embed_ln_bwd", vp, i32, vp, i32, i32, vp, vp, vp, i32, i32, i32, i32, f32, vp)
tap_add = _sig("fm_tap_add", vp, i32, vp, i32, vp, i32, vp, i32, i32, i32, vp)
LPIPS_CHUNK = 64
lpips_stem = _sig("fm_lpips_stem", vp, vp, vp, vp, vp, vp, i32, i32, i32, i32, i32, vp)
lpips_stem_bwd = _sig("fm_lpips_stem_bwd", vp, i32, i32, vp, vp, vp, vp, i32, i32, i32, vp)
maxpool2x2_nhwc = _sig("fm_maxpool2x2_nhwc", vp, i32, vp, i32, i32, i32, i32, i32, i32, vp)
lpips_distance = _sig("fm_lpips_distance", vp, i32, vp, i32, i32, vp, i32, i32, i32, vp, vp, i32, vp, vp)
lpips_tap_bwd = _sig("fm_lpips_tap_bwd", vp, i32, vp, i32, vp, i32, vp, i32, vp, i32, i32, i32, i32, i32, i32, vp)
LOSS_MSE, LOSS_L1, LOSS_SMOOTH_L1, LOSS_CE_INDEX, LOSS_BCE, LOSS_COSINE, LOSS_COSINE_1D = 0, 1, 2, 3, 4, 5, 6
RECONST_CHUNK, EMA_CHUNK, TOKEN_USAGE_MAX_K = 4096, 4096, 1 << 20
reconst_loss_scratch = _sig("fm_reconst_loss_scratch", i32, i32, i32, i64)
reconst_loss = _sig("fm_reconst_loss", vp, vp, i32, i32, i32, i64, vp, vp, vp, vp)
scale_f32 = _sig("fm_scale_f32", vp, vp, i64, vp)
mask_out_samples = _sig("fm_mask_out_samples", vp, vp, f32, vp, i32, i32, i64, vp)
ema_update = _sig("fm_ema_update", vp, i32, i64, f32, f32, vp)
diffusion_pair = _sig("fm_diffusion_pair", vp, vp, vp, vp, vp, i32, vp, vp, i32, i64, vp)
token_usage = _sig("fm_token_usage", vp, i32, i64, i64, i32, vp, vp, vp)
EXPORTS = ["fm_reconst_loss_scratch", "fm_reconst_loss", "fm_scale_f32", "fm_mask_out_samples", "fm_ema_update", "fm_diffusion_pair", "fm_token_usage", "fm_lpips_stem", "fm_lpips_stem_bwd", "fm_maxpool2x2_nhwc", "fm_lpips_distance", "fm_lpips_tap_bwd", "fm_feat_distance", "fm_quick_gelu_bwd", "fm_quick_gelu_bwd_f32", "fm_clip_embed_ln_bwd", "fm_tap_add", "fm_clip_embed_ln", "fm_attn_decode", "fm_vit_patch_rows", "fm_vit_emb_rows", "fm_vit_colsum", "fm_lora_apply", "fm_lora_grad", "fm_vq_assign_wide", "fm_memcodes_assign", "fm_convnext_block", "fm_split3_bf16", "fm_unet_im2col", "fm_groupnorm_nhwc", "fm_add_bf16", "fm_silu_f32_to_bf16", "fm_timestep_embedding", "fm_unet_attention", "fm_diffusion_x0", "fm_quantile_abs",
           "fm_diffusion_step", "fm_unpack_image_u8", "fm_unpack_ids_u16", "fm_unpack_mask_bits", "fm_decoder_attention_from_target", "fm_guidance_combine", "fm_image_mask", "fm_token_budgets", "fm_span_mask", "fm_vq_code_stats", "fm_vq_ema_update", "fm_vq_code_bias", "fm_vq_assign_bias", "fm_vq_code_stats_raw", "fm_vq_ema_update_euclid", "fm_vq_unpatchify", "fm_vq_latent_grad", "fm_tanh_bwd_f32", "fm_embed_rows_f32", "fm_vq_patchify_ex", "fm_vq_cls_emb_bwd", "fm_vq_latent_grad_normalized", "fm_abi_version", "fm_last_error", "fm_gemm_nt", "fm_set_gemm_nt_config", "fm_get_gemm_nt_config", "fm_set_reserved_cus", "fm_get_reserved_cus", "fm_bf16_to_f32_scaled", "fm_add_bf16_f32", "fm_scale_rows_bf16", "fm_gemm_tn", "fm_gemm_tn_multi", "fm_set_gemm_tn_config", "fm_get_gemm_tn_config", "fm_set_tn_transpose_read",
           "fm_get_tn_transpose_read", "fm_layernorm_fwd", "fm_layernorm_fwd_res", "fm_layernorm_bwd", "fm_layernorm_bwd_h", "fm_headnorm_fwd", "fm_headnorm_bwd", "fm_attn_fwd", "fm_attn_bwd",
           "fm_set_attn_transpose_read", "fm_get_attn_transpose_read", "fm_select_embed", "fm_embed_bwd",
           "fm_dense_decoder_mask", "fm_segment_rows", "fm_gather_rows", "fm_cross_entropy", "fm_swiglu_bwd",
           "fm_gelu_bwd", "fm_cast_pad", "fm_transpose_cast_pad", "fm_shadow_refresh", "fm_fold_colscale_grad", "fm_colsum", "fm_f32_to_bf16", "fm_adamw", "fm_adamw_shadow",
           "fm_sumsq", "fm_clip_coef", "fm_vq_patchify", "fm_l2norm_rows", "fm_vq_assign",
           "fm_sample_tokens", "fm_maskgit_commit", "fm_gemm_f32", "fm_attn_f32_fwd", "fm_attn_f32_bwd", "fm_layernorm_bwd_f32", "fm_headnorm_f32_fwd", "fm_headnorm_f32_bwd",
           "fm_swiglu_bwd_f32", "fm_gelu_bwd_f32", "fm_colsum_f32", "fm_cross_entropy_f32", "fm_lab_set",
           "fm_unet_im2col_f32", "fm_groupnorm_nhwc_f32", "fm_unet_attention_f32", "fm_add_f32", "fm_silu_f32", "fm_timestep_embedding_f32",
           "fm_unet_col2im_f32", "fm_groupnorm_nhwc_bwd_f32", "fm_unet_attention_bwd_f32", "fm_silu_bwd_f32"]


def check(rc: int):
    if rc != 0:
        raise RuntimeError(f"libfourm_hip: {lib.fm_last_error().decode()} (rc={rc})")
```

ml-4m_amd/fourm/hip/engine.py:

```python
import math
import os
import random
import weakref
from typing import Dict, List, Optional

import torch
import torch.nn as nn

from . import _lib as L
from . import ops

_WEIGHT_EPOCH = 0
FUSE_ACT_BWD = os.environ.get("FOURM_FUSE_ACT_BWD", "0") == "1"
HEADS_DENSE = os.environ.get("FOURM_HEADS_DENSE", "1") == "1"
HEADS_DENSE_MAX = int(os.environ.get("FOURM_HEADS_DENSE_MAX", "8"))
DEFER_RESIDUAL = os.environ.get("FOURM_DEFER_RESIDUAL", "1") == "1"
HOIST_CTX = os.environ.get("FOURM_HOIST_CTX", "1") == "1"
LN_BWD_FROM_H = os.environ.get("FOURM_LN_BWD_FROM_H", "1") == "1"
DP_RESERVE_ALWAYS = os.environ.get("FOURM_DP_RESERVE_ALWAYS", "0") == "1"


def bump_weight_epoch():
    global _WEIGHT_EPOCH
    _WEIGHT_EPOCH += 1


def ru(x, m):
    return (x + m - 1) // m * m


def is_lora(lin) -> bool:
    return hasattr(lin, "lora_down")


def check_lora_targets(model):
    from fourm.models.lora_utils import MAX_LORA_WIDTH, LoRAWrapper
    ok = set()
    for blk in model.encoder:
        ok |= {id(blk.attn.qkv), id(blk.attn.proj)}
    for blk in getattr(model, "decoder", ()):
        ok |= {id(blk.self_attn.qkv), id(blk.self_attn.proj), id(blk.cross_attn.q), id(blk.cross_attn.kv), id(blk.cross_attn.proj)}
    for name, mod in model.named_modules():
        if not isinstance(mod, LoRAWrapper):
            continue
        if id(mod) not in ok:
            raise NotImplementedError(f"LoRA wrapper at '{name}': the HIP engine adapts the attention Linears of the encoder / decoder blocks only "
                                      "(the MLP's fc1 / fc3 run as one launch whose SwiGLU epilogue consumes the pre-activation; embeddings and "
                                      "heads have no low-rank path)")
        width = mod.lora_down.weight.shape[0]
        if width > MAX_LORA_WIDTH:
            raise NotImplementedError(f"LoRA wrapper at '{name}': rank x packed Linears = {width} exceeds {MAX_LORA_WIDTH}")


class Shadow:
    __slots__ = ("buf", "params", "jobs", "stamp")

    def __init__(self, buf, params, jobs):
        self.buf, self.params, self.jobs, self.stamp = buf, params, jobs, None


class Workspace:

    def __init__(self, device, per_stream: bool = False):
        self.device = device
        self.per_stream = per_stream
        self.bufs: Dict[tuple, torch.Tensor] = {}

    def get(self, name, shape, dtype):
        key = (name, tuple(shape), dtype, torch.cuda.current_stream(self.device).cuda_stream) if self.per_stream else (name, tuple(shape), dtype)
        t = self.bufs.get(key)
        if t is None:
            t = self.bufs[key] = torch.zeros(shape, dtype=dtype, device=self.device)
        return t

    def nbytes(self):
        return sum(t.numel() * t.element_size() for t in self.bufs.values())


def fill_mod_desc(md, d, emb, is_dec: bool, mod_id: int, head_index: int = 0, raw: int = 0, name: str = "modality"):
    kind = emb.kind
    t = d["tensor"]
    B = t.shape[0]
    mask = d["target_mask" if is_dec else "input_mask"]
    mask = mask.reshape(B, -1)
    if mask.dtype != torch.bool:
        mask = mask.bool()
    mask = mask.contiguous()
    keep = [mask]
    md.mask, md.mask_stride = mask.data_ptr(), mask.shape[1]
    md.kind, md.mod_id, md.head_index = kind, mod_id, head_index
    md.pos = emb.pos_emb.data_ptr()
    md.mod_emb = emb.mod_emb.data_ptr()
    md.shifted = 1 if (is_dec and kind == L.KIND_SEQ and raw != 2) else 0
    md.max_len = getattr(emb, "max_length", 0) or 0
    if kind in (L.KIND_TOK, L.KIND_SEQ):
        ids = t.reshape(B, -1)
        if ids.dtype not in (torch.int32, torch.int64):
            ids = ids.long()
        ids = ids.contiguous()
        keep.append(ids)
        md.ids, md.ids_are_i64, md.id_stride = ids.data_ptr(), 1 if ids.dtype == torch.int64 else 0, ids.shape[1]
        md.table = emb.token_emb.weight.data_ptr()
        md.L = ids.shape[1] - (1 if md.shifted else 0)
        if ids.shape[1] != mask.shape[1]:
            raise ValueError(f"{name}: tensor has {ids.shape[1]} positions but the mask has {mask.shape[1]}")
    elif kind == L.KIND_PATCH:
        px = t.float().contiguous()
        keep.append(px)
        _, C, Hh, Ww = px.shape
        ps = emb.patch_size[0]
        md.ids, md.id_stride = px.data_ptr(), C * Hh * Ww
        md.patch, md.channels, md.grid_w = ps, C, Ww // ps
        md.L = (Hh // ps) * (Ww // ps)
    else:
        e = t.float().contiguous()
        keep.append(e)
        md.ids, md.id_stride, md.orig_dim = e.data_ptr(), e.shape[1] * e.shape[2], e.shape[2]
        md.proj_bias = emb.emb_proj.bias.data_ptr()
        md.L = e.shape[1]
    if is_dec and (raw != 2 or "decoder_attention_mask" in d):
        dam = d["decoder_attention_mask"].reshape(B, -1)
        if dam.dtype != torch.int32:
            dam = dam.int()
        dam = dam.contiguous()
        keep.append(dam)
        md.dam = dam.data_ptr()
    return keep


class FourMEngine:
    _pending = None
    _drop_now = None
    drop_uniforms = None

    def __init__(self, model):
        from fourm.models.fm_utils import GatedMlp, NormAttention, act_name
        self.model = model
        check_lora_targets(model)
        self.D = model.dim
        blk = model.encoder[0] if len(model.encoder) else model.decoder[0]
        attn0 = blk.attn if hasattr(blk, "attn") else blk.self_attn
        self.H = attn0.num_heads
        if self.D // self.H != 64:
            raise NotImplementedError(f"head_dim {self.D // self.H}: the HIP attention kernels are built for head_dim 64")
        self.qk_norm = isinstance(attn0, NormAttention)
        self.gated = isinstance(blk.mlp, GatedMlp)
        self.act = act_name(blk.mlp.act)
        if self.gated and self.act != "silu":
            raise NotImplementedError("gated MLP is implemented for SiLU (SwiGLU) only")
        if not self.gated and self.act != "gelu":
            raise NotImplementedError("plain MLP is implemented for exact GELU only")
        self.Hd = blk.mlp.hidden_features
        self.Hp = ru(self.Hd, 64)
        self.scale = 64 ** -0.5
        self.eps = blk.norm1.eps
        prec = getattr(model, "compute_precision", None) or os.environ.get("FOURM_PRECISION", "bf16")
        if prec not in ("bf16", "fp32"):
            raise ValueError(f"compute_precision {prec!r}: 'bf16' or 'fp32'")
        self.fp32 = prec == "fp32"
        self.adt = torch.float32 if self.fp32 else torch.bfloat16
        self.ws: Optional[Workspace] = None
        self.shadows: Dict[tuple, Shadow] = {}
        self._shadow_table = None
        self.flat_params = self.flat_grads = None
        self._slices = {}
        self._ctx = None
        self._dw_jobs = None
        self._pending = None
        self.reducer = None

    @property
    def checkpointing(self):
        return bool(getattr(self.model, "use_act_checkpoint", False))

    @property
    def device(self):
        t = getattr(self.model, "mask_token", None)
        return (t if t is not None else next(self.model.parameters())).device

    def _unique_params(self):
        seen, out = set(), []
        for n, p in getattr(self.model, "engine_parameters", self.model.named_parameters)():
            if id(p) not in seen:
                seen.add(id(p))
                out.append((n, p))
        return out

    def flatten(self):
        named = self._unique_params()
        dev = self.device

        def nodecay(n):
            return "norm." in n or ".norm" in n or n.endswith(".bias")
        late = {id(b.cross_attn.kv.weight) for b in self.model.decoder} if self.hoist_ctx else set()
        named.sort(key=lambda np_: (nodecay(np_[0]), id(np_[1]) in late))
        off, slices = 0, {}
        for n, p in named:
            slices[id(p)] = (off, p.numel())
            off += ru(p.numel(), 16)
        flat = torch.zeros(off, dtype=torch.float32, device=dev)
        for n, p in named:
            o, k = slices[id(p)]
            flat[o:o + k].copy_(p.data.reshape(-1))
            p.data = flat[o:o + k].view(p.shape)
        self.flat_params, self._slices = flat, slices
        self.flat_grads = torch.zeros_like(flat)
        self._named = named
        bump_weight_epoch()

    def _ensure_flat(self):
        if self.flat_params is None or self.flat_params.device != self.device:
            self.flatten()
            return
        for n, p in self._named[:4] + self._named[-4:]:
            o, k = self._slices[id(p)]
            if p.data_ptr() != self.flat_params.data_ptr() + 4 * o:
                self.flatten()
                return

    def grad_stages(self):
        m = self.model
        owner = {}

        def claim(stage, module_or_params):
            ps = module_or_params.parameters() if isinstance(module_or_params, nn.Module) else module_or_params
            for p in ps:
                owner[id(p)] = stage
        for i, blk in enumerate(m.decoder):
            claim(f"dec{i}", blk)
        if self.hoist_ctx:
            claim("dec_emb", [b.cross_attn.kv.weight for b in m.decoder] + [b.context_norm.weight for b in m.decoder])
        claim("heads", [m.decoder_norm.weight] + ([m.decoder_norm.bias] if isinstance(m.decoder_norm.bias, nn.Parameter) else []))
        claim("dec_emb", m.decoder_embeddings)
        claim("dec_emb", [m.mask_token])
        claim("ctx", m.decoder_proj_context)
        claim("ctx", m.encoder_norm)
        for i, blk in enumerate(m.encoder):
            claim(f"enc{i}", blk)
        claim("enc_emb", m.encoder_embeddings)
        if m.register_tokens is not None:
            claim("enc_emb", [m.register_tokens])
        stages = {}
        for n, p in self._named:
            o, k = self._slices[id(p)]
            stage = owner.get(id(p), "enc_emb") if k >= 65536 else "tail"
            stages.setdefault(stage, []).append((o, ru(k, 16)))
        return stages

    def _stage(self, name):
        if self.reducer is not None:
            self.reducer.stage_done(name)

    def grad_view(self, p):
        o, k = self._slices[id(p)]
        return self.flat_grads[o:o + k].view(p.shape)

    def grads_were_cleared(self) -> bool:
        live = getattr(self, "_attached", None)
        if not live:
            return True
        for p in live[:4] + live[-4:]:
            if p.grad is None or p.grad.data_ptr() != self.grad_view(p).data_ptr():
                return True
        return False

    def untouched_params(self):
        c = self._ctx
        if c is None or self.reducer is not None:
            return []
        m, touched, cand = self.model, set(), []
        for names, embs in ((c["enc"]["names"], m.encoder_embeddings), (c["dec"]["names"], m.decoder_embeddings)):
            for n, e in embs.items():
                if n in names:
                    touched.update(id(p) for p in e.parameters())
                else:
                    cand.extend(e.parameters())
        return [p for p in cand if id(p) not in touched]

    def attach_grads(self, zero: bool, untouched=()):
        if zero:
            with ops._prof("fills"):
                self.flat_grads.zero_()
            self._window_touched = set()
        skip = {id(p) for p in untouched} - getattr(self, "_window_touched", set())
        self._attached = []
        for n, p in self._named:
            if not p.requires_grad:
                continue
            if id(p) in skip:
                p.grad = None
                continue
            self._window_touched.add(id(p))
            p.grad = self.grad_view(p)
            self._attached.append(p)

    def _stamp(self, params):
        return tuple((p._version, _WEIGHT_EPOCH, p.data_ptr()) for p in params)

    def _get_shadow(self, key, make) -> torch.Tensor:
        s = self.shadows.get(key)
        if s is None:
            s = self.shadows[key] = make()
            for p in s.params:
                regs = getattr(p, "_fourm_shadows", None)
                if regs is None:
                    regs = p._fourm_shadows = []
                regs.append((weakref.ref(self), key))
        if s.stamp != self._stamp(s.params):
            self._refresh_shadows()
        return s.buf

    def _refresh_shadows(self):
        stale = [s for s in self.shadows.values() if s.stamp != self._stamp(s.params)]
        jobs = []
        for s in stale:
            jobs += [(j[0].detach().reshape(j[0].shape[0], -1), j[1], j[2], j[3].detach() if len(j) > 3 and j[3] is not None else None) for j in s.jobs]
        sig = tuple((a.data_ptr(), b.data_ptr(), tr, sc.data_ptr() if sc is not None else 0) for (a, b, tr, sc) in jobs)
        if self._shadow_table is None or self._shadow_table[0] != sig:
            table, tiles = ops.shadow_jobs_table(jobs, self.device)
            self._shadow_table = (sig, table, len(jobs), tiles)
        _, table, n, tiles = self._shadow_table
        ops.shadow_refresh(table, n, tiles)
        for s in stale:
            s.stamp = self._stamp(s.params)

    def mark_shadows_fresh(self, keys, written):
        for key in keys:
            s = self.shadows.get(key)
            if s is not None and all(len(j) == 3 and (id(j[0]), j[1].data_ptr()) in written for j in s.jobs):
                s.stamp = self._stamp(s.params)

    def w(self, p, pad_rows=False):
        if self.fp32:
            return p.detach().reshape(p.shape[0], -1)
        def make():
            out_f, in_f = p.shape[0], p[0].numel()
            buf = torch.zeros(ru(out_f, 64) if pad_rows else out_f, ru(in_f, 64), dtype=torch.bfloat16, device=p.device)
            return Shadow(buf, (p,), [(p, buf, False)])
        s = self._get_shadow(("w", id(p)), make)
        assert not pad_rows or s.shape[0] >= ru(p.shape[0], 64), "w(): the cached image was created without pad_rows"
        return s

    def wt(self, p, pad_rows=False):
        if self.fp32:
            return p.detach().reshape(p.shape[0], -1).t()
        def make():
            out_f, in_f = p.shape[0], p[0].numel()
            buf = torch.zeros(ru(in_f, 64) if pad_rows else in_f, ru(out_f, 64), dtype=torch.bfloat16, device=p.device)
            return Shadow(buf, (p,), [(p, buf, True)])
        s = self._get_shadow(("wt", id(p)), make)
        assert not pad_rows or s.shape[0] >= ru(p[0].numel(), 64), "wt(): the cached image was created without pad_rows"
        return s

    def w_fold(self, lin, norm):
        p, g = lin.weight, norm.weight
        def make():
            out_f, in_f = p.shape
            buf = torch.zeros(out_f, in_f if self.fp32 else ru(in_f, 64), dtype=self.adt, device=p.device)
            return Shadow(buf, (p, g), [(p, buf, False, g)])
        return self._get_shadow(("wfold", id(p)), make)

    def wt_fold_stack(self):
        m, D = self.model, self.D
        def make():
            Ld = len(m.decoder)
            buf = torch.zeros(D, Ld * 2 * D, dtype=self.adt, device=self.device)
            ps, jobs = [], []
            for i, blk in enumerate(m.decoder):
                p, g = blk.cross_attn.kv.weight, blk.context_norm.weight
                ps += [p, g]
                jobs.append((p, buf[:, i * 2 * D:(i + 1) * 2 * D], True, g))
            return Shadow(buf, tuple(ps), jobs)
        return self._get_shadow(("wtfold", 0), make)

    @property
    def hoist_ctx(self):
        h = getattr(self, "_hoist_ctx", None)
        if h is None:
            dec = getattr(self.model, "decoder", ())
            h = HOIST_CTX and len(dec) > 0 and all(
                not isinstance(b.context_norm.bias, nn.Parameter) and b.cross_attn.kv.bias is None and not is_lora(b.cross_attn.kv)
                for b in dec)
            self._hoist_ctx = h
        return h

    def w13t(self, mlp):
        def make():
            buf = torch.zeros(self.D, 2 * self.Hp, dtype=torch.bfloat16, device=self.device)
            p1, p3 = mlp.fc1.weight, mlp.fc3.weight
            return Shadow(buf, (p1, p3), [(p1, buf[:, :self.Hp], True), (p3, buf[:, self.Hp:], True)])
        return self._get_shadow(("w13t", id(mlp)), make)

    def _mod_desc(self, md: L.ModDesc, name, d, emb, is_dec, head_index=0, raw=0):
        return fill_mod_desc(md, d, emb, is_dec, int(self.model.modality_info[name]["id"]), head_index, raw, name)

    def select(self, mod_dict, n_keep: int, is_dec: bool, order: List[str], prefix: str, want_x0=True, heads=None, raw=0):
        m = self.model
        embs = m.decoder_embeddings if is_dec else m.encoder_embeddings
        names = [n for n in order if n in embs]
        if not names:
            raise ValueError("no modality of mod_dict is known to the model")
        if len(names) > L.FM_MAX_MODS:
            raise ValueError(f"{len(names)} modalities exceed FM_MAX_MODS={L.FM_MAX_MODS}")
# ... 266 lines not shown
    def decoder_mask(self, cs, mod_pre):
        m = self.model
        return dict(mask_kind=L.MASK_DECODER, cs=None if m.decoder_causal_mask else cs, causal=m.decoder_causal_mask,
                    modq=mod_pre if m.decoder_sep_mask else None, modk=mod_pre if m.decoder_sep_mask else None)

    def encode_context(self, enc, st=None):
        m = self.model
        save = st is not None
        B, N = enc["B"], enc["Nt"]
        emask = self.keypad(enc["mask"])
        x = enc["x0"]
        ckpt = save and self.checkpointing
        for i, blk in enumerate(m.encoder):
            if ckpt:
                st["enc_layers"].append(dict(ckpt_in=x))
                x = self.encoder_block_fwd(blk, x, B, N, emask, None, f"enc{i % 2}", defer_out=True, out_name=f"enc{i}.x_out")
                st["enc_layers"][-1]["dp"] = self._last_dp
                continue
            sv = {} if save else None
            x = self.encoder_block_fwd(blk, x, B, N, emask, sv, f"enc{i}" if save else f"enc{i % 2}", defer_out=True)
            if save:
                st["enc_layers"].append(sv)
        R, Rp, D = B * N, x.shape[0], self.D
        sv_top = {} if save else None
        xn = self._ln(m.encoder_norm, x, self._buf(sv_top, "top", "xn", (Rp, D), self.adt), R, sv_top, "en", "top")
        ctx = self._buf(sv_top, "top", "ctx", (Rp, D), torch.float32)
        pc = m.decoder_proj_context
        ops.gemm_nt(xn, self.w(pc.weight), ctx, epilogue=L.EPI_RESIDUAL, res=enc["emb"], bias=pc.bias, M=R, N=D, K=D)
        return x, ctx, emask, sv_top

    def trunk_forward(self, enc, dec, save: bool):
        m = self.model
        B, N, Mt = enc["B"], enc["Nt"], dec["Nt"]
        st = dict(enc_layers=[], dec_layers=[]) if save else None
        x, ctx, emask, sv_top = self.encode_context(enc, st)
        y = dec["x0"]
        smask = self.decoder_mask(dec["cs"], dec["mod_pre"]) if "cs" in dec else dec["sa_mask"]
        ctx_hat, sv_hat = None, None
        if self.hoist_ctx:
            sv_hat = {} if save else None
            ctx_hat = self._ln(self._unit_norm(), ctx, self._buf(sv_hat, "top", "ctx_hat", (ctx.shape[0], self.D), self.adt), B * N, sv_hat, "ch", "top")
        for i, blk in enumerate(m.decoder):
            if save and self.checkpointing:
                st["dec_layers"].append(dict(ckpt_in=y))
                y = self.decoder_block_fwd(blk, y, ctx, B, Mt, N, smask, emask, None, f"dec{i % 2}", defer_out=i + 1 < len(m.decoder),
                                           out_name=f"dec{i}.y_out", ctx_hat=ctx_hat)
                st["dec_layers"][-1]["dp"] = self._last_dp
                continue
            sv = {} if save else None
            y = self.decoder_block_fwd(blk, y, ctx, B, Mt, N, smask, emask, sv, f"dec{i}" if save else f"dec{i % 2}",
                                       defer_out=i + 1 < len(m.decoder), ctx_hat=ctx_hat)
            if save:
                st["dec_layers"].append(sv)
        if save:
            st.update(top=sv_top, x_final=x, y_final=y, ctx=ctx, emask=emask, smask=smask, ctx_hat=ctx_hat, sv_hat=sv_hat)
        return y, st

    def heads_setup(self, dec, y_final, save):
        m = self.model
        heads = dec["heads"]
        nH = len(heads)
        B, Mt, D = dec["B"], dec["Nt"], self.D
        R = B * Mt
        Rp = ops.padded_rows(R, nH)
        ws, dev, i32 = self.ws, self.device, torch.int32
        hs = dict(n=nH, Rp=Rp, heads=heads)
        hs["seg_start"], hs["seg_count"] = ws.get("heads.seg_start", (nH,), i32), ws.get("heads.seg_count", (nH,), i32)
        hs["perm"], hs["r2p"] = ws.get("heads.perm", (Rp,), i32), ws.get("heads.r2p", (R,), i32)
        hs["tile_group"] = ws.get("heads.tile_group", (Rp // ops.SEG,), i32)
        ops.segment_rows(dec["head_of_row"].view(-1), nH, hs["seg_start"], hs["seg_count"], hs["perm"], hs["r2p"], hs["tile_group"])
        sv = {} if save else None
        yp = ws.get("heads.yp", (Rp, D), self.adt)
        with ops._prof("fills"):
            yp.zero_()
        self._ln(m.decoder_norm, y_final, yp, R, sv, "dn", "heads", row_map=hs["r2p"])
        vocabs = [m.decoder_embeddings[h].vocab_size for h in heads]
        hs["vocabs"], hs["maxV"] = vocabs, max(vocabs)
        ldl = ru(hs["maxV"], 64)
        w_fwd = [self.w(m.decoder_embeddings[h].to_logits.weight) for h in heads]
        w_bwd = [self.wt(m.decoder_embeddings[h].to_logits.weight) for h in heads] if save else None
        key = tuple(t.data_ptr() for t in w_fwd) + (tuple(t.data_ptr() for t in w_bwd) if save else ())
        cache = getattr(self, "_head_groups", None)
        if cache is None or cache[0] != key:
            fwd = ops.make_groups([dict(W=t, N=v, K=D, ldw=D) for t, v in zip(w_fwd, vocabs)], dev)
            if self.fp32:
                bwd = ops.make_groups([dict(W=m.decoder_embeddings[h].to_logits.weight, N=D, K=v, ldw=D, transposed=1)
                                       for h, v in zip(heads, vocabs)], dev) if save else None
            else:
                bwd = ops.make_groups([dict(W=t, N=D, K=ru(v, 64), ldw=ru(v, 64)) for t, v in zip(w_bwd, vocabs)], dev) if save else None
            vt = torch.tensor(vocabs, dtype=i32, device=dev)
            self._head_groups = cache = (key, fwd, bwd, vt)
        hs["g_fwd"], hs["g_bwd"], hs["vocab_t"] = cache[1], cache[2], cache[3]
        logits = ws.get("heads.logits", (Rp, ldl), self.adt)
        if HEADS_DENSE and not self.fp32 and nH <= HEADS_DENSE_MAX and ops.heads_dense_ok(w_fwd, vocabs, logits):
            ops.gemm_nt_heads(yp, w_fwd, vocabs, hs["seg_start"], hs["seg_count"], logits, D)
        else:
            ops.gemm_nt_grouped(yp, hs["g_fwd"], hs["tile_group"], logits, hs["maxV"], max_K=D)
        hs.update(yp=yp, logits=logits, sv=sv)
        hs["row_loss"] = ws.get("heads.row_loss", (Rp,), torch.float32)
        hs["row_lse"] = ws.get("heads.row_lse", (Rp,), torch.float32)
        hs["head_loss"] = ws.get("heads.head_loss", (nH,), torch.float32)
        hs["total"] = ws.get("heads.total", (1,), torch.float32)
        return hs

    def loss_forward(self, dec, hs, loss_type):
        lt = L.LOSS_MOD if loss_type in ("mod", "modality") else L.LOSS_TOKEN
        hs["loss_type"] = lt
        ops.cross_entropy(hs["logits"], hs["perm"], hs["tile_group"], dec["target_ids"].view(-1), hs["vocab_t"], hs["seg_start"],
                          hs["seg_count"], hs["n"], hs["maxV"], hs["row_loss"], hs["row_lse"], hs["head_loss"], hs["total"], loss_type=lt)
        return hs["total"], hs["head_loss"]

    def dec_order(self, mod_dict):
        names = [n for n in mod_dict if n in self.model.decoder_embeddings]
        return random.sample(names, len(names))

    def train_forward(self, mod_dict, n_enc, n_dec, loss_type, save=True):
        if loss_type not in ("mod", "modality", "token"):
            raise ValueError("Invalid loss type")
        self.prepare()
        if save:
            self._ensure_flat()
        enc_names = [n for n in mod_dict if n in self.model.encoder_embeddings]
        enc = self.select(mod_dict, n_enc, False, enc_names, "enc.")
        dec = self.select(mod_dict, n_dec, True, self.dec_order(mod_dict), "dec.")
        y, st = self.trunk_forward(enc, dec, save)
        hs = self.heads_setup(dec, y, save)
        total, head_loss = self.loss_forward(dec, hs, loss_type)
        if save:
            self._ctx = dict(enc=enc, dec=dec, st=st, hs=hs)
        return total, head_loss, hs["heads"], hs["seg_count"]

    def _g(self, p):
        return self.grad_view(p) if p.requires_grad else None

    def _dW(self, dy, x, lin, R64, n_cols=None, dy_cols=None):
        g = self._g(lin.weight)
        N = lin.weight.shape[0] if n_cols is None else n_cols
        if g is not None:
            if self._dw_jobs is not None:
                self._dw_jobs.append((dy, x, g.view(g.shape[0], -1), N, lin.weight[0].numel(), R64))
            else:
                ops.gemm_tn(dy, x, g.view(g.shape[0], -1), N=N, K=lin.weight[0].numel(), R=R64)
        if lin.bias is not None and lin.bias.requires_grad:
            ops.colsum(dy, self.grad_view(lin.bias), N, R=R64)

    def _flush_dW(self):
        jobs, self._dw_jobs = self._dw_jobs, None
        if jobs:
            ops.gemm_tn_multi(jobs)

    def _ln_bwd(self, norm, dy, x, sv, key, g, g_bf, R, dres, dy_row_map=None):
        dw = self._g(norm.weight)
        db = self._g(norm.bias) if isinstance(norm.bias, nn.Parameter) else None
        ops.layernorm_bwd(dy, x, norm.weight, sv[key + ".mu"], sv[key + ".rs"], g, dres=dres, dx_bf16=g_bf, dw=dw, db=db,
                          dy_row_map=dy_row_map, R=R, h=sv.get(key + ".h"))

    def _mlp_bwd(self, mlp, sv, g_bf, R, Rp):
        bf, D, Hp, Hd = self.adt, self.D, self.Hp, self.Hd
        R64 = R
        ws = self.ws
        self._dW(g_bf, sv["act"], mlp.fc2, R64)
        dh = ws.get("bwd.dh", (Rp, D), bf)
        fuse = FUSE_ACT_BWD and self.act != "quick_gelu"
        if not fuse:
            da = ws.get("bwd.da", (Rp, Hp), bf)
            padN = not self.fp32 and Hp != Hd
            ops.gemm_nt(g_bf, self.wt(mlp.fc2.weight, padN), da, M=R, N=Hp if padN else Hd, K=D)
        if self.gated:
            dgu = ws.get("bwd.dgu", (Rp, 2 * Hp), bf)
            if fuse:
                ops.gemm_nt(g_bf, self.wt(mlp.fc2.weight), dgu, M=R, N=Hd, K=D, epilogue=L.EPI_SWIGLU_BWD, res=sv["gu"], Hp=Hp)
            else:
                ops.swiglu_bwd(da, sv["gu"], dgu, Hd, Hp, R=R)
            self._dW(dgu[:, :Hp], sv["h2"], mlp.fc1, R64, n_cols=Hd)
            self._dW(dgu[:, Hp:], sv["h2"], mlp.fc3, R64, n_cols=Hd)
            if self.fp32:
                ops.gemm_nt(dgu[:, :Hp], self.wt(mlp.fc1.weight), dh, M=R, N=D, K=Hd)
                ops.gemm_nt(dgu[:, Hp:], self.wt(mlp.fc3.weight), dh, M=R, N=D, K=Hd, epilogue=L.EPI_F32, res=dh)
            else:
                ops.gemm_nt(dgu, self.w13t(mlp), dh, M=R, N=D, K=2 * Hp)
        else:
            dpre = ws.get("bwd.dpre", (Rp, Hp), bf)
            if fuse:
                ops.gemm_nt(g_bf, self.wt(mlp.fc2.weight), dpre, M=R, N=Hd, K=D, epilogue=L.EPI_GELU_BWD, res=sv["pre"])
            elif self.act == "quick_gelu":
                ops.quick_gelu_bwd(da, sv["pre"], dpre, Hd, Hp, R=R)
            else:
                ops.gelu_bwd(da, sv["pre"], dpre, Hd, Hp, R=R)
            self._dW(dpre, sv["h2"], mlp.fc1, R64, n_cols=Hd)
            ops.gemm_nt(dpre, self.wt(mlp.fc1.weight), dh, M=R, N=D, K=Hp)
        return dh

    def _self_attn_bwd(self, attn, sv, g_bf, B, N, R, Rp, mask):
        bf, D = self.adt, self.D
        R64, ws = R, self.ws
        self._dW(g_bf, sv["o"], attn.proj, R64)
        do = ws.get("bwd.do", (Rp, D), bf)
        ops.gemm_nt(g_bf, self.wt(attn.proj.weight), do, M=R, N=D, K=D)
        self._lora_bwd(attn.proj, g_bf, sv["o"], do, sv.get("lora.proj"), R)
        dqkv = ws.get("bwd.dqkv", (Rp, 3 * D), bf)
        qkv = sv["qkv"]
        if self.qk_norm:
            dqkn = ws.get("bwd.dqkn", (Rp, 2 * D), bf)
            ops.attn_bwd(sv["qkn.q"], sv["qkn.k"], qkv[:, 2 * D:], sv["o"], do, dqkn[:, :D], dqkn[:, D:], dqkv[:, 2 * D:],
                         B, self.H, N, N, self.scale, sv["sm"], sv["sl"], zero_attn=getattr(attn, "allow_zero_attn", False), **mask)
            self._qk_norm_bwd(attn, sv, "qkn", dqkn[:, :D], dqkn[:, D:], qkv[:, :D], qkv[:, D:2 * D], dqkv[:, :D], dqkv[:, D:2 * D], R, R)
        else:
            ops.attn_bwd(qkv[:, :D], qkv[:, D:2 * D], qkv[:, 2 * D:], sv["o"], do, dqkv[:, :D], dqkv[:, D:2 * D], dqkv[:, 2 * D:],
                         B, self.H, N, N, self.scale, sv["sm"], sv["sl"], zero_attn=getattr(attn, "allow_zero_attn", False), **mask)
        self._dW(dqkv, sv["h1"], attn.qkv, R64)
        dh = ws.get("bwd.dh", (Rp, D), bf)
        ops.gemm_nt(dqkv, self.wt(attn.qkv.weight), dh, M=R, N=D, K=3 * D)
        self._lora_bwd(attn.qkv, dqkv, sv["h1"], dh, sv.get("lora.qkv"), R)
        return dh

    def encoder_block_bwd(self, blk, sv, g, g_bf, B, N, mask):
        R, Rp = B * N, g.shape[0]
        self._dw_jobs = []
        dp = sv.get("dp")
        if dp:
            ops.scale_rows_bf16(g_bf, dp[1], N, R)
        dh = self._mlp_bwd(blk.mlp, sv, g_bf, R, Rp)
        g1 = self.ws.get("bwd.enc.gbf1", tuple(g_bf.shape), g_bf.dtype)
        self._ln_bwd(blk.norm2, dh, sv["x_mid"], sv, "n2", g, g1, R, dres=g)
        if dp:
            ops.scale_rows_bf16(g1, dp[0], N, R)
        dh = self._self_attn_bwd(blk.attn, sv, g1, B, N, R, Rp, mask)
        self._flush_dW()
        self._ln_bwd(blk.norm1, dh, sv["x_in"], sv, "n1", g, g_bf, R, dres=g)

    def decoder_block_bwd(self, blk, sv, g, g_bf, dctx, dctx_bf, ctx, B, M, N, sa_mask, xa_mask, hoist=None):
        bf, D = self.adt, self.D
        Rq, Rqp, Rc, Rcp = B * M, g.shape[0], B * N, ctx.shape[0]
        ws = self.ws
        self._dw_jobs = []
        g_in = g_bf
        dp = sv.get("dp")
        if dp:
            ops.scale_rows_bf16(g_in, dp[2], M, Rq)
        dh = self._mlp_bwd(blk.mlp, sv, g_in, Rq, Rqp)
        g_bf = ws.get("bwd.dec.gbf1", tuple(g_in.shape), g_in.dtype)
        self._ln_bwd(blk.norm2, dh, sv["y2"], sv, "n2", g, g_bf, Rq, dres=g)
        if dp:
            ops.scale_rows_bf16(g_bf, dp[1], M, Rq)
        xa = blk.cross_attn
        self._dW(g_bf, sv["o2"], xa.proj, Rq)
        do = ws.get("bwd.do", (Rqp, D), bf)
        ops.gemm_nt(g_bf, self.wt(xa.proj.weight), do, M=Rq, N=D, K=D)
        self._lora_bwd(xa.proj, g_bf, sv["o2"], do, sv.get("lora.proj2"), Rq)
        dq = ws.get("bwd.dq", (Rqp, D), bf)
        dkv = ws.get("bwd.dkv", (Rcp, 2 * D), bf) if hoist is None else hoist[0]
        kv = sv["kv"]
        if self.qk_norm:
            dqn = ws.get("bwd.dqn", (Rqp, D), bf)
            dkn = ws.get("bwd.dkn", (Rcp, D), bf)
            ops.attn_bwd(sv["xqkn.q"], sv["xqkn.k"], kv[:, D:], sv["o2"], do, dqn, dkn, dkv[:, D:], B, self.H, M, N, self.scale,
                         sv["sm2"], sv["sl2"], zero_attn=getattr(xa, "allow_zero_attn", False), **xa_mask)
            self._qk_norm_bwd(xa, sv, "xqkn", dqn, dkn, sv["q"], kv[:, :D], dq, dkv[:, :D], Rq, Rc)
        else:
            ops.attn_bwd(sv["q"], kv[:, :D], kv[:, D:], sv["o2"], do, dq, dkv[:, :D], dkv[:, D:], B, self.H, M, N, self.scale,
                         sv["sm2"], sv["sl2"], zero_attn=getattr(xa, "allow_zero_attn", False), **xa_mask)
        self._dW(dq, sv["hq"], xa.q, Rq)
        dhq = ws.get("bwd.dh", (Rqp, D), bf)
        ops.gemm_nt(dq, self.wt(xa.q.weight), dhq, M=Rq, N=D, K=D)
        self._lora_bwd(xa.q, dq, sv["hq"], dhq, sv.get("lora.q"), Rq)
        g_bf = ws.get("bwd.dec.gbf2", tuple(g_in.shape), g_in.dtype)
        self._ln_bwd(blk.query_norm, dhq, sv["y1"], sv, "nq", g, g_bf, Rq, dres=g)
        if dp:
            ops.scale_rows_bf16(g_bf, dp[0], M, Rq)
        if hoist is None:
            self._dW(dkv, sv["hc"], xa.kv, Rc)
            dhc = ws.get("bwd.dhc", (Rcp, D), bf)
            ops.gemm_nt(dkv, self.wt(xa.kv.weight), dhc, M=Rc, N=D, K=2 * D)
            self._lora_bwd(xa.kv, dkv, sv["hc"], dhc, sv.get("lora.kv"), Rc)
            self._ln_bwd(blk.context_norm, dhc, ctx, sv, "nc", dctx, dctx_bf, Rc, dres=dctx)
        elif xa.kv.weight.requires_grad or blk.context_norm.weight.requires_grad:
            self._dw_jobs.append((dkv, hoist[1], hoist[2], 2 * D, D, Rc))
        dh = self._self_attn_bwd(blk.self_attn, sv, g_bf, B, M, Rq, Rqp, sa_mask)
        self._flush_dW()
        self._ln_bwd(blk.norm1, dh, sv["y_in"], sv, "n1", g, g_in, Rq, dres=g)

    def _embed_bwd(self, sel, dx, dx_extra, is_dec):
        m = self.model
        embs = m.decoder_embeddings if is_dec else m.encoder_embeddings
        d = L.EmbedBwdDesc()
        for i, n in enumerate(sel["names"]):
            e, md = embs[n], d.mods[i]
            md.kind = e.kind
            if e.kind in (L.KIND_TOK, L.KIND_SEQ) and not (is_dec and e.kind == L.KIND_TOK):
                w = e.token_emb.weight
                md.d_table = self.grad_view(w).data_ptr() if w.requires_grad else None
                pad = e.token_emb.padding_idx
                md.has_padding_idx, md.padding_idx = (1, pad) if pad is not None else (0, 0)
            if isinstance(e.pos_emb, nn.Parameter) and e.pos_emb.requires_grad:
                md.d_pos = self.grad_view(e.pos_emb).data_ptr()
            if e.mod_emb.requires_grad:
                md.d_mod_emb = self.grad_view(e.mod_emb).data_ptr()
            if e.kind == L.KIND_SEQ_EMB and e.emb_proj.bias.requires_grad:
                md.d_proj_bias = self.grad_view(e.emb_proj.bias).data_ptr()
        d.dx, d.lddx = dx.data_ptr(), dx.stride(0)
        d.slot_mod, d.slot_src, d.slot_pos = sel["slot_mod"].data_ptr(), sel["slot_src"].data_ptr(), sel["slot_pos"].data_ptr()
        if is_dec and m.mask_token.requires_grad:
            d.d_mask_token = self.grad_view(m.mask_token).data_ptr()
        if not is_dec and m.num_register_tokens and m.register_tokens.requires_grad:
            d.d_reg_tokens = self.grad_view(m.register_tokens).data_ptr()
        d.n_mods, d.batch, d.dim, d.Nt, d.is_decoder = len(sel["names"]), sel["B"], self.D, sel["Nt"], 1 if is_dec else 0
        with ops._prof("embed_bwd"):
            L.check(L.embed_bwd(ops.C.byref(d), ops._stream()))
        if dx_extra is not None:
            d2 = L.EmbedBwdDesc()
            ops.C.memmove(ops.C.byref(d2), ops.C.byref(d), ops.C.sizeof(d))
            for i in range(d.n_mods):
                d2.mods[i].d_table = None
                d2.mods[i].d_proj_bias = None
            d2.d_reg_tokens = None
            d2.dx, d2.lddx = dx_extra.data_ptr(), dx_extra.stride(0)
            with ops._prof("embed_bwd"):
                L.check(L.embed_bwd(ops.C.byref(d2), ops._stream()))

    def train_backward(self, grad_scale: torch.Tensor):
        c = self._ctx
        if c is None:
            raise RuntimeError("train_backward without a preceding training forward")
        self._ctx, self._dw_jobs = None, None
        if self.reducer is not None:
            self.reducer.begin()
            if getattr(self.reducer, "reserved_cus", 0):
                L.lib.fm_set_reserved_cus(int(self.reducer.reserved_cus))
        m, ws = self.model, self.ws
        enc, dec, st, hs = c["enc"], c["dec"], c["st"], c["hs"]
        B, N, Mt, D = enc["B"], enc["Nt"], dec["Nt"], self.D
        bf, f32 = self.adt, torch.float32
        Rq, Rc = B * Mt, B * N
        Rqp, Rcp = st["y_final"].shape[0], st["x_final"].shape[0]
        ops.cross_entropy(hs["logits"], hs["perm"], hs["tile_group"], dec["target_ids"].view(-1), hs["vocab_t"], hs["seg_start"],
                          hs["seg_count"], hs["n"], hs["maxV"], hs["row_loss"], hs["row_lse"], hs["head_loss"], hs["total"],
                          loss_type=hs["loss_type"], grad_scale=grad_scale, write_grad=True)
        dyp = ws.get("bwd.dyp", (hs["Rp"], D), bf)
        ops.gemm_nt_grouped(hs["logits"], hs["g_bwd"], hs["tile_group"], dyp, D, max_K=ru(hs["maxV"], 64))
        heads = [m.decoder_embeddings[h] for h in hs["heads"]]
        if any(h.to_logits.weight.requires_grad for h in heads):
            outs = [self.grad_view(h.to_logits.weight) if h.to_logits.weight.requires_grad else None for h in heads]
            key = tuple(o.data_ptr() if o is not None else 0 for o in outs)
            cache = getattr(self, "_head_tn_groups", None)
            if cache is None or cache[0] != key:
                cache = self._head_tn_groups = (key, ops.make_groups(
                    [dict(out=o, N=(v if o is not None else 0)) for o, v in zip(outs, hs["vocabs"])], self.device))
            tn = cache[1]
            ops.gemm_tn_grouped(hs["logits"], hs["yp"], tn, hs["seg_start"], hs["seg_count"], hs["n"], hs["maxV"], hs["Rp"], D)
        g = ws.get("bwd.g_dec", (Rqp, D), f32)
        g_bf = ws.get("bwd.g_dec_bf", (Rqp, D), bf)
        self._ln_bwd(m.decoder_norm, dyp, st["y_final"], hs["sv"], "dn", g, g_bf, Rq, dres=None, dy_row_map=hs["r2p"])
        self._stage("heads")
        dctx = ws.get("bwd.dctx", (Rcp, D), f32)
        dctx_bf = ws.get("bwd.dctx_bf", (Rcp, D), bf)
        Ld = len(m.decoder)
        ctx_hat = st.get("ctx_hat")
        if ctx_hat is None:
            with ops._prof("fills"):
                dctx.zero_()
        else:
            dkv_all = ws.get("bwd.dkv_all", (Rcp, Ld * 2 * D), bf)
            dwp = ws.get("bwd.dwp", (Ld, 2 * D, D), f32)
            with ops._prof("fills"):
                dwp.zero_()
        for i in reversed(range(Ld)):
            sv = st["dec_layers"][i]
            if "ckpt_in" in sv:
                y_in, dp, sv = sv["ckpt_in"], sv["dp"], {}
                self.decoder_block_fwd(m.decoder[i], y_in, st["ctx"], B, Mt, N, st["smask"], st["emask"], sv, "ckpt", out_name="ckpt.out", dp=dp,
                                       ctx_hat=ctx_hat)
            hoist = None if ctx_hat is None else (dkv_all[:, i * 2 * D:(i + 1) * 2 * D], ctx_hat, dwp[i])
            self.decoder_block_bwd(m.decoder[i], sv, g, g_bf, dctx, dctx_bf, st["ctx"], B, Mt, N, st["smask"], st["emask"], hoist=hoist)
            self._stage(f"dec{i}")
        if ctx_hat is not None and Ld:
            dxh = ws.get("bwd.dhc", (Rcp, D), bf)
            ops.gemm_nt(dkv_all, self.wt_fold_stack(), dxh, M=Rc, N=D, K=Ld * 2 * D)
            self._ln_bwd(self._unit_norm(), dxh, st["ctx"], st["sv_hat"], "ch", dctx, dctx_bf, Rc, dres=None)
            jobs = [(dwp[i], b.cross_attn.kv.weight.detach(), b.context_norm.weight.detach(), self._g(b.cross_attn.kv.weight), self._g(b.context_norm.weight))
                    for i, b in enumerate(m.decoder) if b.cross_attn.kv.weight.requires_grad or b.context_norm.weight.requires_grad]
            if jobs:
                ops.fold_colscale_grad(jobs)
        self._embed_bwd(dec, g, None, True)
        self._stage("dec_emb")
        top = st["top"]
        if len(m.decoder) == 0:
            ops.f32_to_bf16(dctx, dctx_bf)
        self._dW(dctx_bf, top["xn"], m.decoder_proj_context, Rc)
        dxn = ws.get("bwd.dh", (Rcp, D), bf)
        ops.gemm_nt(dctx_bf, self.wt(m.decoder_proj_context.weight), dxn, M=Rc, N=D, K=D)
        ge = ws.get("bwd.g_enc", (Rcp, D), f32)
        ge_bf = ws.get("bwd.g_enc_bf", (Rcp, D), bf)
        self._ln_bwd(m.encoder_norm, dxn, st["x_final"], top, "en", ge, ge_bf, Rc, dres=None)
        self._stage("ctx")
        for i in reversed(range(len(m.encoder))):
            sv = st["enc_layers"][i]
            if "ckpt_in" in sv:
                x_in, dp, sv = sv["ckpt_in"], sv["dp"], {}
                self.encoder_block_fwd(m.encoder[i], x_in, B, N, st["emask"], sv, "ckpt", out_name="ckpt.out", dp=dp)
            self.encoder_block_bwd(m.encoder[i], sv, ge, ge_bf, B, N, st["emask"])
            self._stage(f"enc{i}")
        for n in enc["names"]:
            e = m.encoder_embeddings[n]
            if e.kind == L.KIND_PATCH and e.proj.weight.requires_grad:
                ops.gemm_tn(ge_bf, enc["patch_rows"], self.grad_view(e.proj.weight), N=D, K=e.proj.weight.shape[1], R=Rc)
            elif e.kind == L.KIND_SEQ_EMB and e.emb_proj.weight.requires_grad:
                ops.gemm_tn(ge_bf, enc["seqemb_rows"], self.grad_view(e.emb_proj.weight), N=D, K=e.emb_proj.weight.shape[1], R=Rc)
        self._embed_bwd(enc, ge, dctx, False)
        if self.reducer is not None:
            self.reducer.finish()
            if getattr(self.reducer, "reserved_cus", 0) and not DP_RESERVE_ALWAYS:
                L.lib.fm_set_reserved_cus(0)
```

ml-4m_amd/fourm/hip/ops.py:

```python
import contextlib
import ctypes as C
import threading
from typing import Optional

import torch

from . import _lib as L

_PROFILER = None


def set_profiler(p):
    global _PROFILER
    _PROFILER = p


class _Null:
    def __enter__(self):
        return self

    def __exit__(self, *a):
        return False


# ... 112 lines not shown
    if w2 is not None:
        assert w2.stride() == w.stride()
    a.ldo, a.ldo2, a.ldr = out.stride(0), out2.stride(0) if out2 is not None else 0, res.stride(0) if res is not None else 0
    a.Hp, a.epilogue, a.accumulate = Hp, epilogue, 1 if accumulate else 0
    with _prof("gemm_f32", 2.0 * a.M * a.N * a.K * (2 if epilogue == L.EPI_SWIGLU else 1), 4.0 * (a.K * (a.M + a.N) + a.M * a.N), tag=f"M{a.M} N{a.N} K{a.K}"):
        L.check(L.gemm_f32(C.byref(a), _stream()))
    return out


@_timed("heads_gemm_nt (logits, dY)")
def gemm_nt_grouped(x, groups, tile_group, out, max_N, M=None, max_K=0):
    if x.dtype == torch.float32:
        a = L.GemmF32Args()
        a.X, a.out, a.groups, a.tile_group = _p(x), _p(out), _p(groups), _p(tile_group)
        a.M, a.N, a.max_N, a.seg_rows = (x.shape[0] if M is None else M), max_N, max_N, SEG
        a.sxm, a.sxk, a.ldo, a.epilogue = x.stride(0), 1, out.stride(0), L.EPI_BF16
        L.check(L.gemm_f32(C.byref(a), _stream()))
        return out
    a = L.GemmNTArgs()
    a.X, a.out = _p(x), _p(out)
    a.M = x.shape[0] if M is None else M
    a.K = max_K
    a.ldx, a.ldo = _ld(x), _ld(out)
    a.epilogue = L.EPI_BF16
    a.groups, a.tile_group, a.max_N = _p(groups), _p(tile_group), max_N
    L.check(L.gemm_nt(C.byref(a), _stream()))
    return out


def heads_dense_ok(ws, vocabs, out):
    return (out.dtype == torch.bfloat16 and all(v % 8 == 0 for v in vocabs) and all(w.dtype == torch.bfloat16 and w.shape[1] % 64 == 0 for w in ws)
            and _ld(out) % 64 == 0 and out.data_ptr() % 128 == 0)


@_timed("heads_gemm_nt (logits, dY)")
def gemm_nt_heads(x, ws, vocabs, seg_start, seg_count, out, K):
    for h, (w, v) in enumerate(zip(ws, vocabs)):
        a = L.GemmNTArgs()
        a.W, a.X, a.out = _p(w), _p(x), _p(out)
        a.M, a.N, a.K = x.shape[0], v, K
        a.ldw, a.ldx, a.ldo = _ld(w), _ld(x), _ld(out)
        a.epilogue = L.EPI_BF16
        a.m_dev, a.row0_dev = seg_count.data_ptr() + 4 * h, seg_start.data_ptr() + 4 * h
        L.check(L.gemm_nt(C.byref(a), _stream()))
    return out


def gemm_tn(a_mat, b_mat, out, *, N=None, K=None, R=None, splits=0, force_tr=-1, a_cols=0, b_cols=0):
    if a_mat.dtype == torch.float32:
        g = L.GemmF32Args()
        g.X, g.W, g.out = _p(a_mat), _p(b_mat), _p(out)
        g.M = a_mat.shape[1] if N is None else N
        g.N = b_mat.shape[1] if K is None else K
        g.K = a_mat.shape[0] if R is None else R
        g.sxm, g.sxk, g.swn, g.swk = 1, a_mat.stride(0), 1, b_mat.stride(0)
        g.ldo, g.epilogue, g.accumulate = _ld(out), L.EPI_BF16, 1
        L.check(L.gemm_f32(C.byref(g), _stream()))
        return out
    a = L.GemmTNArgs()
    a.A, a.B, a.out = _p(a_mat), _p(b_mat), _p(out)
    a.R = a_mat.shape[0] if R is None else R
    a.N = a_mat.shape[1] if N is None else N
    a.K = b_mat.shape[1] if K is None else K
    a.lda, a.ldb, a.ldo = _ld(a_mat), _ld(b_mat), _ld(out)
    a.a_cols = a_cols or a_mat.shape[1]
    a.b_cols = b_cols or b_mat.shape[1]
    a.splits, a.force_tr = splits, force_tr
    with _prof("gemm_tn", 2.0 * a.R * a.N * a.K, 2.0 * a.R * (a.N + a.K) + 4.0 * a.N * a.K, tag=f"R{a.R} N{a.N} K{a.K}"):
        L.check(L.gemm_tn(C.byref(a), _stream()))
    return out


def gemm_tn_multi(jobs):
    if not jobs:
        return
    if jobs[0][0].dtype == torch.float32:
        for a_mat, b_mat, out, N, K, R in jobs:
            gemm_tn(a_mat, b_mat, out, N=N, K=K, R=R)
        return
    for lo in range(0, len(jobs), L.TN_MAX_JOBS):
        part = jobs[lo:lo + L.TN_MAX_JOBS]
        arr = (L.GemmTNJob * len(part))()
        flops = 0.0
        for j, (a_mat, b_mat, out, N, K, R) in zip(arr, part):
            j.A, j.B, j.out = _p(a_mat), _p(b_mat), _p(out)
            j.R, j.N, j.K = R, N, K
            j.lda, j.ldb, j.ldo = _ld(a_mat), _ld(b_mat), _ld(out)
            j.a_cols, j.b_cols = a_mat.shape[1], b_mat.shape[1]
            flops += 2.0 * R * N * K
        with _prof("gemm_tn_multi", flops, 0.0, tag=f"jobs{len(part)} R{part[0][5]}"):
            L.check(L.gemm_tn_multi(arr, len(part), _stream()))


@_timed("heads_gemm_tn (dW)")
def gemm_tn_grouped(a_mat, b_mat, groups, seg_start, seg_count, n_groups, max_N, max_R, K, *, splits=0, force_tr=-1):
    if a_mat.dtype == torch.float32:
        g = L.GemmF32Args()
        g.X, g.W, g.groups, g.seg_start, g.seg_count = _p(a_mat), _p(b_mat), _p(groups), _p(seg_start), _p(seg_count)
        g.N, g.max_N, g.n_groups = K, max_N, n_groups
        g.sxm, g.sxk, g.swn, g.swk = 1, a_mat.stride(0), 1, b_mat.stride(0)
        g.ldo, g.epilogue, g.accumulate = K, L.EPI_BF16, 1
        L.check(L.gemm_f32(C.byref(g), _stream()))
        return
    a = L.GemmTNArgs()
    a.A, a.B = _p(a_mat), _p(b_mat)
    a.K = K
    a.lda, a.ldb, a.ldo = _ld(a_mat), _ld(b_mat), K
    a.a_cols, a.b_cols = a_mat.shape[1], b_mat.shape[1]
    a.splits, a.force_tr = splits, force_tr
    a.groups, a.seg_start, a.seg_count = _p(groups), _p(seg_start), _p(seg_count)
    a.n_groups, a.max_N, a.max_R = n_groups, max_N, max_R
    L.check(L.gemm_tn(C.byref(a), _stream()))


def make_groups(entries, device):
    arr = (L.GemmGroup * len(entries))()
    for i, e in enumerate(entries):
        arr[i].W = e["W"].data_ptr() if e.get("W") is not None else None
        arr[i].out = e["out"].data_ptr() if e.get("out") is not None else None
        arr[i].N, arr[i].K, arr[i].ldw = e["N"], e.get("K", 0), e.get("ldw", 0)
        arr[i].pad_ = e.get("transposed", 0)
    host = torch.frombuffer(bytearray(bytes(arr)), dtype=torch.uint8)
    return host.to(device)


def layernorm_fwd(x, w, b, y, mean=None, rstd=None, row_map=None, eps=1e-6, R=None, delta=None, x_out=None):
    R = x.shape[0] if R is None else R
    if delta is not None:
        with _prof("layernorm_fwd", 0.0, R * w.numel() * (10 + y.element_size())):
            L.check(L.layernorm_fwd_res(_p(x), _ld(x), _p(delta), _ld(delta), _p(x_out), _ld(x_out), _p(w), _p(b), _p(y), _ld(y),
                                        1 if y.dtype == torch.float32 else 0, _p(mean), _p(rstd), _p(row_map), R, w.numel(), eps, _stream()))
        return y
    with _prof("layernorm_fwd", 0.0, R * w.numel() * (4 + y.element_size())):
        return _ln_fwd(x, w, b, y, mean, rstd, row_map, eps, R)


def _ln_fwd(x, w, b, y, mean, rstd, row_map, eps, R):
    L.check(L.layernorm_fwd(_p(x), _ld(x), _p(w), _p(b), _p(y), _ld(y), 1 if y.dtype == torch.float32 else 0,
                            _p(mean), _p(rstd), _p(row_map), R, w.numel(), eps, _stream()))
    return y


def layernorm_bwd(dy, x, w, mean, rstd, dx, *, dres=None, dx_bf16=None, dw=None, db=None, dy_row_map=None, R=None, h=None):
    R = x.shape[0] if R is None else R
    if h is not None and dy.dtype != torch.float32 and db is None and dy_row_map is None:
        with _prof("layernorm_bwd", 0.0, R * w.numel() * (2 + 2 + 4 + 4 + (2 if dx_bf16 is not None else 0))):
            L.check(L.layernorm_bwd_h(_p(dy), _ld(dy), _p(h), _ld(h), _p(x), _ld(x), _p(w), _p(mean), _p(rstd), _p(dres), _p(dx), _ld(dx),
                                      _p(dx_bf16), _ld(dx_bf16) if dx_bf16 is not None else 0, _p(dw), R, w.numel(), _stream()))
        return dx
    with _prof("layernorm_bwd", 0.0, R * w.numel() * (2 + 4 + 4 + 4 + (2 if dx_bf16 is not None else 0))):
        return _ln_bwd(dy, x, w, mean, rstd, dx, dres, dx_bf16, dw, db, dy_row_map, R)


def _ln_bwd(dy, x, w, mean, rstd, dx, dres, dx_bf16, dw, db, dy_row_map, R):
    if dy.dtype == torch.float32:
        L.check(L.layernorm_bwd_f32(_p(dy), _ld(dy), _p(dy_row_map), _p(x), _ld(x), _p(w), _p(mean), _p(rstd), _p(dres), _p(dx), _ld(dx),
                                    _p(dx_bf16), _ld(dx_bf16) if dx_bf16 is not None else 0, _p(dw), _p(db), R, w.numel(), _stream()))
        return dx
    L.check(L.layernorm_bwd(_p(dy), _ld(dy), _p(dy_row_map), _p(x), _ld(x), _p(w), _p(mean), _p(rstd), _p(dres), _p(dx), _ld(dx),
                            _p(dx_bf16), _ld(dx_bf16) if dx_bf16 is not None else 0, _p(dw), _p(db), R, w.numel(), _stream()))
    return dx


@_timed("headnorm")
def headnorm_fwd(x, w, b, y, stats, R, H, eps):
    if x.dtype == torch.float32:
        return L.check(L.headnorm_f32_fwd(_p(x), _ld(x), _p(w), _p(b), _p(y), _ld(y), _p(stats), R, H, eps, _stream()))
    L.check(L.headnorm_fwd(_p(x), _ld(x), _p(w), _p(b), _p(y), _ld(y), _p(stats), R, H, eps, _stream()))


@_timed("headnorm")
def headnorm_bwd(dy, x, w, stats, dx, dw, db, R, H):
    if x.dtype == torch.float32:
        return L.check(L.headnorm_f32_bwd(_p(dy), _ld(dy), _p(x), _ld(x), _p(w), _p(stats), _p(dx), _ld(dx), _p(dw), _p(db), R, H, _stream()))
    L.check(L.headnorm_bwd(_p(dy), _ld(dy), _p(x), _ld(x), _p(w), _p(stats), _p(dx), _ld(dx), _p(dw), _p(db), R, H, _stream()))


def _attn_args(q, k, v, o, B, H, Nq, Nk, scale, mask_kind, kpad, cs, modq, modk, dense, causal, stat_m, stat_l, force_tr, zero_attn=False):
    a = L.AttnArgs()
    a.Q, a.K, a.V, a.O = _p(q), _p(k), _p(v), _p(o)
    a.ldq, a.ldk, a.ldv, a.ldo = q.stride(0), k.stride(0), v.stride(0), o.stride(0)
    a.B, a.H, a.Nq, a.Nk, a.head_dim, a.mask_kind = B, H, Nq, Nk, 64, mask_kind
    a.scale, a.causal = scale, 1 if causal else 0
    a.kpad, a.cs, a.modq, a.modk, a.dense = _p(kpad), _p(cs), _p(modq), _p(modk), _p(dense)
    a.stat_m, a.stat_l = _p(stat_m), _p(stat_l)
    a.force_tr, a.zero_attn = force_tr, 1 if zero_attn else 0
    return a


def attn_fwd(q, k, v, o, B, H, Nq, Nk, scale, *, mask_kind=L.MASK_NONE, kpad=None, cs=None, modq=None, modk=None, dense=None,
             causal=False, stat_m=None, stat_l=None, force_tr=-1, kv_batch_rows=0, zero_attn=False):
    a = _attn_args(q, k, v, o, B, H, Nq, Nk, scale, mask_kind, kpad, cs, modq, modk, dense, causal, stat_m, stat_l, force_tr, zero_attn)
    a.kv_batch_rows = kv_batch_rows
    if q.dtype == torch.float32:
        L.check(L.attn_f32_fwd(C.byref(a), _stream()))
        return o
    with _prof("attn_fwd", 4.0 * B * H * Nq * Nk * 64):
        L.check(L.attn_fwd(C.byref(a), _stream()))
    return o


@_timed("attn_decode")
def attn_decode(q, k, v, o, B, H, Nk, scale, *, kv_batch_rows=0, k_new_row=-1, q_norm=None, k_norm=None, eps=1e-6, kpad=None, zero_attn=False):
    a = L.AttnDecodeArgs()
    a.q, a.k, a.v, a.o = _p(q), _p(k), _p(v), _p(o)
    if not (q.dtype == k.dtype == v.dtype == o.dtype) or q.dtype not in (torch.bfloat16, torch.float32):
        raise TypeError("attn_decode: q, k, v, o must share one of bf16 / fp32")
    for w in (q_norm or ()) + (k_norm or ()):
        if w is not None and (w.dtype != torch.float32 or w.numel() != 64 or not w.is_contiguous()):
            raise TypeError("attn_decode: norm vectors are contiguous fp32 (64)")
    a.q_w, a.q_b = (_p(q_norm[0]), _p(q_norm[1])) if q_norm is not None else (None, None)
    a.k_w, a.k_b = (_p(k_norm[0]), _p(k_norm[1])) if k_norm is not None else (None, None)
    if kpad is not None and (kpad.dtype not in (torch.bool, torch.uint8) or kpad.shape != (B, Nk) or not kpad.is_contiguous()):
        raise TypeError("attn_decode: kpad is a contiguous (B, Nk) bool / uint8 tensor")
    a.kpad = _p(kpad)
    a.ldq, a.ldk, a.ldv, a.ldo = _ld(q), _ld(k), _ld(v), _ld(o)
    a.B, a.H, a.Nk, a.kv_batch_rows, a.k_new_row = B, H, Nk, kv_batch_rows, k_new_row
    a.is_f32, a.zero_attn, a.scale, a.eps = int(q.dtype == torch.float32), 1 if zero_attn else 0, scale, eps
    L.check(L.attn_decode(C.byref(a), _stream()))
    return o


def attn_bwd(q, k, v, o, do, dq, dk, dv, B, H, Nq, Nk, scale, stat_m, stat_l, *, mask_kind=L.MASK_NONE, kpad=None, cs=None,
             modq=None, modk=None, dense=None, causal=False, force_tr=-1, zero_attn=False):
    a = _attn_args(q, k, v, o, B, H, Nq, Nk, scale, mask_kind, kpad, cs, modq, modk, dense, causal, stat_m, stat_l, force_tr, zero_attn)
    a.dO, a.dQ, a.dK, a.dV = _p(do), _p(dq), _p(dk), _p(dv)
    a.lddo, a.lddq, a.lddk, a.lddv = do.stride(0), dq.stride(0), dk.stride(0), dv.stride(0)
    if q.dtype == torch.float32:
        dk.zero_(); dv.zero_()
        L.check(L.attn_f32_bwd(C.byref(a), _stream()))
        return
    with _prof("attn_bwd", 10.0 * B * H * Nq * Nk * 64):
        L.check(L.attn_bwd(C.byref(a), _stream()))


def padded_rows(R: int, n_heads: int) -> int:
    return ru(R, SEG) + SEG * (n_heads - 1)


@_timed("heads_misc")
def segment_rows(head_of_row, n_heads, seg_start, seg_count, perm, row_to_padded, tile_group):
    L.check(L.segment_rows(_p(head_of_row), head_of_row.numel(), n_heads, _p(seg_start), _p(seg_count), _p(perm),
                           _p(row_to_padded), _p(tile_group), perm.numel(), _stream()))


@_timed("heads_misc")
def gather_rows(src, perm, dst, D):
    L.check(L.gather_rows(_p(src), _ld(src), _p(perm), _p(dst), _ld(dst), perm.numel(), D, _stream()))


@_timed("cross_entropy")
def cross_entropy(logits, perm, tile_group, target_ids, vocab, seg_start, seg_count, n_heads, max_vocab, row_loss, row_lse, head_loss,
                  total_loss, *, loss_type=L.LOSS_MOD, grad_scale=None, write_grad=False):
    fn = L.cross_entropy_f32 if logits.dtype == torch.float32 else L.cross_entropy
    L.check(fn(_p(logits), _ld(logits), _p(perm), _p(tile_group), _p(target_ids), _p(vocab), _p(seg_start),
                            _p(seg_count), _p(grad_scale), loss_type, n_heads, perm.numel(), max_vocab, _p(row_loss), _p(row_lse),
                            _p(head_loss), _p(total_loss), 1 if write_grad else 0, _stream()))


@_timed("swiglu_bwd")
def swiglu_bwd(da, gu, dgu, H, Hp, R=None):
    if da.dtype == torch.float32:
        return L.check(L.swiglu_bwd_f32(_p(da), _ld(da), _p(gu), _ld(gu), _p(dgu), _ld(dgu), da.shape[0] if R is None else R, H, Hp, _stream()))
    L.check(L.swiglu_bwd(_p(da), _ld(da), _p(gu), _ld(gu), _p(dgu), _ld(dgu), da.shape[0] if R is None else R, H, Hp, _stream()))


@_timed("gelu_bwd")
def gelu_bwd(dh, pre, dpre, H, Hp, R=None):
    if dh.dtype == torch.float32:
        return L.check(L.gelu_bwd_f32(_p(dh), _ld(dh), _p(pre), _ld(pre), _p(dpre), _ld(dpre), dh.shape[0] if R is None else R, H, _stream()))
    L.check(L.gelu_bwd(_p(dh), _ld(dh), _p(pre), _ld(pre), _p(dpre), _ld(dpre), dh.shape[0] if R is None else R, H, Hp, _stream()))


@_timed("gelu_bwd")
def quick_gelu_bwd(da, pre, dpre, H, Hp, R=None):
    R = da.shape[0] if R is None else R
    if da.dtype == torch.float32:
        return L.check(L.quick_gelu_bwd_f32(_p(da), _ld(da), _p(pre), _ld(pre), _p(dpre), _ld(dpre), R, H, _stream()))
    L.check(L.quick_gelu_bwd(_p(da), _ld(da), _p(pre), _ld(pre), _p(dpre), _ld(dpre), R, H, Hp, _stream()))


def tap_add(g, dtap, g_bf=None, row_scale=None, rows_per_sample=0, R=None):
    R = g.shape[0] if R is None else R
    L.check(L.tap_add(_p(g), _ld(g), _p(g_bf), _ld(g_bf) if g_bf is not None else 0, _p(dtap), _ld(dtap), _p(row_scale), rows_per_sample, R, g.shape[1],
                      _stream()))
    return g


def feat_distance(pred, tgt, B, T, mode, loss, dpred):
    L.check(L.feat_distance(_p(pred), _ld(pred), _p(tgt), _ld(tgt), B, T, pred.shape[1], mode, _p(loss), _p(dpred), _ld(dpred), _stream()))
    return loss


def _is_f32(t):
    if t.dtype not in (torch.float32, torch.bfloat16):
        raise TypeError(f"feature rows are bf16 or f32, got {t.dtype}")
    return 1 if t.dtype == torch.float32 else 0


def lpips_stem(img, mul, add, w, bias, out, B, H, W):
    esz = out.element_size()
    with _prof("lpips_stem", 2.0 * B * H * W * 64 * 27, B * H * W * (12.0 + 64 * esz), tag=f"B{B} {H}x{W}"):
        L.check(L.lpips_stem(_p(img), _p(mul), _p(add), _p(w), _p(bias), _p(out), _ld(out), _is_f32(out), B, H, W, _stream()))
    return out


# ... 294 lines not shown
```

Baseline: 1.178 million tokens/s.

## Replace layernorm-backward weight-grad atomics with per-block partials and batched reduction

LayerNorm backward now writes each block's dw/db sums to a partial buffer instead of atomically adding them into the gradient. The partials are reduced in one batched kernel at each reducer stage boundary and at the end of backward. This removes contention from many blocks hitting the same D addresses, at the cost of extra workspace, additional memory traffic and a deferred reduction launch. Separately, the embedding-backward kernel is restructured to use 1024-thread blocks covering several batch rows, per-lane scalar columns, and wave-wide prefetch of slot metadata read through readlane.

```diff
diff --git a/include/fourm_hip.h b/include/fourm_hip.h
--- a/include/fourm_hip.h
+++ b/include/fourm_hip.h
@@ -75,6 +75,16 @@
 int fm_layernorm_bwd_h(const void* dy, int lddy, const void* h, int ldh, const void* x, int ldx, const void* w,
                        const void* mean, const void* rstd, const void* dres, void* dx, int lddx, void* dx_bf16,
                        int lddxbf, void* dw, int R, int D, void* stream);
+int fm_layernorm_bwd_partial_rows(int R);
+int fm_layernorm_bwd_partial(const void* dy, int lddy, const int32_t* dy_row_map, const void* h, int ldh, const void* x, int ldx,
+                             const void* w, const void* mean, const void* rstd, const void* dres, void* dx, int lddx, void* dx_bf16,
+                             int lddxbf, void* pw, void* pb, int partial_rows, int R, int D, void* stream);
+#define FM_LN_REDUCE_MAX_JOBS 128
+typedef struct fm_ln_reduce_job {
+    const void* partial; void* dst;
+    int32_t n_partial, D;
+} fm_ln_reduce_job;
+int fm_ln_reduce_partials(const fm_ln_reduce_job* jobs, int n_jobs, void* stream);
 
 int fm_headnorm_fwd(const void* x, int ldx, const void* w, const void* b, void* y, int ldy, void* stats, int R, int H, float eps,
                     void* stream);
diff --git a/ml-4m_amd/csrc/layernorm.hip b/ml-4m_amd/csrc/layernorm.hip
--- a/ml-4m_amd/csrc/layernorm.hip
+++ b/ml-4m_amd/csrc/layernorm.hip
@@ -130,7 +130,8 @@
                                                      const float* __restrict__ x, int ldx, const float* __restrict__ w,
                                                      const float* __restrict__ mean, const float* __restrict__ rstd,
                                                      const float* dres, float* dx, int lddx, bf16_t* __restrict__ dx_bf, int lddxbf,
-                                                     float* __restrict__ dw, float* __restrict__ db, int R, int D, int BWD_ROWS, int nt_dx) {
+                                                     float* __restrict__ dw, float* __restrict__ db, int R, int D, int BWD_ROWS, int nt_dx,
+                                                     float* __restrict__ pw, float* __restrict__ pb) {
     extern __shared__ __attribute__((aligned(16))) char smem[];
     float* red = (float*)smem;
     const int lane = threadIdx.x & 63, wave = threadIdx.x >> 6;
@@ -218,7 +219,7 @@
             }
         }
     }
-    if (!dw && !db) return;
+    if (!dw && !db && !pw && !pb) return;
 #pragma unroll
     for (int c = 0; c < MAXC; ++c) {
         const int ch = lane + 64 * c;
@@ -229,9 +230,36 @@
     }
     __syncthreads();
     for (int i = threadIdx.x; i < D; i += 256) {
-        if (dw) unsafeAtomicAdd(dw + i, (red[i] + red[D + i]) + (red[2 * D + i] + red[3 * D + i]));
-        if constexpr (HAS_DB) if (db) unsafeAtomicAdd(db + i, (red[4 * D + i] + red[5 * D + i]) + (red[6 * D + i] + red[7 * D + i]));
-    }
+        const float sw = (red[i] + red[D + i]) + (red[2 * D + i] + red[3 * D + i]);
+        if (pw) pw[(size_t)blockIdx.x * D + i] = sw;
+        else if (dw) unsafeAtomicAdd(dw + i, sw);
+        if constexpr (HAS_DB) {
+            const float sb = (red[4 * D + i] + red[5 * D + i]) + (red[6 * D + i] + red[7 * D + i]);
+            if (pb) pb[(size_t)blockIdx.x * D + i] = sb;
+            else if (db) unsafeAtomicAdd(db + i, sb);
+        }
+    }
+}
+
+struct LnReduceArgs {
+    fm_ln_reduce_job j[FM_LN_REDUCE_MAX_JOBS];
+};
+__global__ __launch_bounds__(256) void ln_reduce_kernel(LnReduceArgs a) {
+    __shared__ float red[4][64];
+    const fm_ln_reduce_job& job = a.j[blockIdx.y];
+    const int D = job.D, n = job.n_partial;
+    if ((int)blockIdx.x * 64 >= D) return;
+    const int lane = threadIdx.x & 63, wave = threadIdx.x >> 6;
+    const int c = blockIdx.x * 64 + lane;
+    const float* src = (const float*)job.partial;
+    float s = 0.f;
+    if (c < D) {
+#pragma unroll 8
+        for (int p = wave; p < n; p += 4) s += src[(size_t)p * D + c];
+    }
+    red[wave][lane] = s;
+    __syncthreads();
+    if (wave == 0 && c < D) unsafeAtomicAdd((float*)job.dst + c, (red[0][lane] + red[1][lane]) + (red[2][lane] + red[3][lane]));
 }
 
 
@@ -363,13 +391,15 @@
 
 static int layernorm_bwd_launch(const void* dy, int lddy, const int32_t* dy_row_map, const void* h, int ldh, const void* x, int ldx, const void* w,
                                 const void* mean, const void* rstd, const void* dres, void* dx, int lddx, void* dx_bf16,
-                                int lddxbf, void* dw, void* db, int R, int D, void* stream) {
+                                int lddxbf, void* dw, void* db, int R, int D, void* stream, void* pw = nullptr, void* pb = nullptr,
+                                int partial_rows = 0) {
     FM_CHECK_ARG(dy && x && w && mean && rstd && dx, "fm_layernorm_bwd: null pointer");
     FM_CHECK_ARG(!h || ldh % 4 == 0, "fm_layernorm_bwd_h: ldh must be a multiple of 4");
     FM_CHECK_ARG(R > 0 && D > 0 && D % 4 == 0 && D <= 64 * 4 * MAXC_LIMIT, "fm_layernorm_bwd: D=%d unsupported", D);
     FM_CHECK_ARG(ldx % 4 == 0 && lddy % 4 == 0 && lddx % 4 == 0 && lddxbf % 4 == 0, "fm_layernorm_bwd: leading dims must be multiples of 4");
     const int BWD_ROWS = bwd_rows(R);
     const int grid = (R + BWD_ROWS - 1) / BWD_ROWS;
+    FM_CHECK_ARG((!pw && !pb) || partial_rows >= grid, "fm_layernorm_bwd_partial: %d partial rows lent, %d needed (fm_layernorm_bwd_partial_rows)", partial_rows, grid);
     const size_t lds = (size_t)8 * D * sizeof(float);
 #define LN_BWD_(C, FH)                                                                                                      \
     {                                                                                                                       \
@@ -378,7 +408,7 @@
         (void)once;                                                                                                         \
         hipLaunchKernelGGL(k, dim3(grid), dim3(256), lds, (hipStream_t)stream, (const bf16_t*)dy, lddy, dy_row_map, (const bf16_t*)h, ldh, \
                            (const float*)x, ldx, (const float*)w, (const float*)mean, (const float*)rstd, (const float*)dres, (float*)dx, lddx, \
-                           (bf16_t*)dx_bf16, lddxbf, (float*)dw, (float*)db, R, D, BWD_ROWS, ((ln_nt_flags() >> 1) & 1) | ((ln_nt_flags() >> 2) & 2) | ((ln_nt_flags() >> 2) & 4));                               \
+                           (bf16_t*)dx_bf16, lddxbf, (float*)dw, (float*)db, R, D, BWD_ROWS, ((ln_nt_flags() >> 1) & 1) | ((ln_nt_flags() >> 2) & 2) | ((ln_nt_flags() >> 2) & 4), (float*)pw, (float*)pb);                               \
     }
 #define LN_BWD(C) { if (h) LN_BWD_(C, true) else LN_BWD_(C, false) }
     switch (chunks_for(D)) {
@@ -404,6 +434,32 @@
                                   int lddxbf, void* dw, int R, int D, void* stream) {
     FM_CHECK_ARG(h, "fm_layernorm_bwd_h: null pointer");
     return layernorm_bwd_launch(dy, lddy, nullptr, h, ldh, x, ldx, w, mean, rstd, dres, dx, lddx, dx_bf16, lddxbf, dw, nullptr, R, D, stream);
+}
+
+extern "C" int fm_layernorm_bwd_partial_rows(int R) { return R > 0 ? (R + bwd_rows(R) - 1) / bwd_rows(R) : 0; }
+
+extern "C" int fm_layernorm_bwd_partial(const void* dy, int lddy, const int32_t* dy_row_map, const void* h, int ldh, const void* x, int ldx,
+                                        const void* w, const void* mean, const void* rstd, const void* dres, void* dx, int lddx, void* dx_bf16,
+                                        int lddxbf, void* pw, void* pb, int partial_rows, int R, int D, void* stream) {
+    FM_CHECK_ARG(pw, "fm_layernorm_bwd_partial: no partial buffer");
+    FM_CHECK_ARG(!h || (!dy_row_map && !pb), "fm_layernorm_bwd_partial: the form that reads h takes no row map and has no bias gradient");
+    return layernorm_bwd_launch(dy, lddy, dy_row_map, h, ldh, x, ldx, w, mean, rstd, dres, dx, lddx, dx_bf16, lddxbf, nullptr, nullptr, R, D, stream,
+                                pw, pb, partial_rows);
+}
+
+extern "C" int fm_ln_reduce_partials(const fm_ln_reduce_job* jobs, int n_jobs, void* stream) {
+    FM_CHECK_ARG(jobs && n_jobs > 0, "fm_ln_reduce_partials: no jobs");
+    for (int i = 0; i < n_jobs; ++i)
+        FM_CHECK_ARG(jobs[i].partial && jobs[i].dst && jobs[i].n_partial > 0 && jobs[i].D > 0, "fm_ln_reduce_partials: job %d incomplete", i);
+    for (int j0 = 0; j0 < n_jobs; j0 += FM_LN_REDUCE_MAX_JOBS) {
+        LnReduceArgs a{};
+        const int n = std::min(n_jobs - j0, (int)FM_LN_REDUCE_MAX_JOBS);
+        int max_d = 0;
+        for (int i = 0; i < n; ++i) { a.j[i] = jobs[j0 + i]; max_d = std::max(max_d, a.j[i].D); }
+        hipLaunchKernelGGL(ln_reduce_kernel, dim3((max_d + 63) / 64, n), dim3(256), 0, (hipStream_t)stream, a);
+    }
+    FM_CHECK_LAUNCH("fm_ln_reduce_partials");
+    return 0;
 }
 
 extern "C" int fm_headnorm_fwd(const void* x, int ldx, const void* w, const void* b, void* y, int ldy, void* stats, int R, int H, float eps,
diff --git a/ml-4m_amd/csrc/select_embed.hip b/ml-4m_amd/csrc/select_embed.hip
--- a/ml-4m_amd/csrc/select_embed.hip
+++ b/ml-4m_amd/csrc/select_embed.hip
@@ -246,76 +246,91 @@
     }
 }
 
-__global__ __launch_bounds__(256) void embed_bwd_kernel(fm_embed_bwd_desc d) {
+template <int NK>
+__global__ __launch_bounds__(1024) void embed_bwd_kernel(fm_embed_bwd_desc d) {
     extern __shared__ __attribute__((aligned(16))) char smem[];
     float* acc = (float*)smem;
-    const int D = d.dim, nch = D >> 2;
-    const int b = blockIdx.x, lane = threadIdx.x & 63, wave = threadIdx.x >> 6;
+    const int D = d.dim;
+    const int lane = threadIdx.x & 63, wave = __builtin_amdgcn_readfirstlane(threadIdx.x >> 6);
+    const int b = blockIdx.x * (blockDim.x >> 8) + (wave >> 2);
     const int rows = d.n_mods + 1;
-    for (int i = threadIdx.x; i < rows * D; i += 256) acc[i] = 0.f;
+    for (int i = threadIdx.x; i < rows * D; i += blockDim.x) acc[i] = 0.f;
     __shared__ int used[FM_MAX_MODS + 1];
     if (threadIdx.x <= FM_MAX_MODS) used[threadIdx.x] = 0;
     __syncthreads();
-    constexpr int MAXQ = 8;
-    const int parts = 4 * gridDim.y, part = wave + 4 * blockIdx.y;
-    const int per = (d.Nt + parts - 1) / parts, s_lo = part * per, s_hi = min(d.Nt, s_lo + per);
-    float4 racc[MAXQ];
+    const int parts = 4 * gridDim.y, part = (wave & 3) + 4 * blockIdx.y;
+    const int per = (d.Nt + parts - 1) / parts, s_lo = part * per, s_hi = b < d.batch ? min(d.Nt, s_lo + per) : s_lo;
+    float racc[NK];
     int cur = -1;
     bool cur_mask = false;
     auto flush = [&]() {
         if (cur < 0) return;
 #pragma unroll
-        for (int q = 0; q < MAXQ; ++q) {
-            const int c = lane + 64 * q;
-            if (c >= nch) break;
-            float* a0 = acc + (size_t)cur * D + c * 4;
-            atomicAdd(a0, racc[q].x); atomicAdd(a0 + 1, racc[q].y); atomicAdd(a0 + 2, racc[q].z); atomicAdd(a0 + 3, racc[q].w);
-            if (cur_mask) {
-                float* a1 = acc + (size_t)d.n_mods * D + c * 4;
-                atomicAdd(a1, racc[q].x); atomicAdd(a1 + 1, racc[q].y); atomicAdd(a1 + 2, racc[q].z); atomicAdd(a1 + 3, racc[q].w);
+        for (int k = 0; k < NK; ++k) {
+            const int c = lane + 64 * k;
+            if (c < D) {
+                atomicAdd(acc + (size_t)cur * D + c, racc[k]);
+                if (cur_mask) atomicAdd(acc + (size_t)d.n_mods * D + c, racc[k]);
             }
         }
     };
-    for (int s = s_lo; s < s_hi; ++s) {
-        const size_t row = (size_t)b * d.Nt + s;
-        const int m = ((const int32_t*)d.slot_mod)[row];
-        if (m == -1) continue;
-        const float* g = (const float*)d.dx + row * d.lddx;
-        if (m == -2) {
-            if (d.d_reg_tokens)
-                for (int c = lane; c < D; c += 64) unsafeAtomicAdd((float*)d.d_reg_tokens + (size_t)s * D + c, g[c]);
-            continue;
-        }
-        const fm_embed_bwd_mod& md = d.mods[m];
-        const int src = ((const int32_t*)d.slot_src)[row];
-        const int posrow = ((const int32_t*)d.slot_pos)[row];
-        const bool to_mask_token = d.is_decoder && md.kind == FM_KIND_TOK;
-        if (m != cur) {
-            flush();
-            cur = m; cur_mask = to_mask_token;
-#pragma unroll
-            for (int q = 0; q < MAXQ; ++q) racc[q] = make_float4(0.f, 0.f, 0.f, 0.f);
-            if (lane == 0) { used[m] = 1; if (to_mask_token) used[d.n_mods] = 1; }
-        }
-        float* trow = nullptr;
-        if (to_mask_token) {}
-        else if ((md.kind == FM_KIND_TOK || md.kind == FM_KIND_SEQ) && md.d_table && !(md.has_padding_idx && src == md.padding_idx))
-            trow = (float*)md.d_table + (size_t)src * D;
-        else if (md.kind == FM_KIND_SEQ_EMB && md.d_proj_bias) trow = (float*)md.d_proj_bias;
-        float* prow = md.d_pos ? (float*)md.d_pos + (size_t)posrow * D : nullptr;
-#pragma unroll
-        for (int q = 0; q < MAXQ; ++q) {
-            const int c = lane + 64 * q;
-            if (c >= nch) break;
-            const float4 v = *(const float4*)(g + c * 4);
-            racc[q].x += v.x; racc[q].y += v.y; racc[q].z += v.z; racc[q].w += v.w;
+    for (int base = s_lo; base < s_hi; base += 64) {
+        int l_mod = -1, l_src = 0, l_pos = 0;
+        if (base + lane < s_hi) {
+            const size_t row = (size_t)b * d.Nt + base + lane;
+            l_mod = ((const int32_t*)d.slot_mod)[row];
+            l_src = ((const int32_t*)d.slot_src)[row];
+            l_pos = ((const int32_t*)d.slot_pos)[row];
+        }
+        const int cnt = min(64, s_hi - base);
+        for (int i = 0; i < cnt; ++i) {
+            const int m = __builtin_amdgcn_readlane(l_mod, i);
+            if (m == -1) continue;
+            const int s = base + i;
+            const float* g = (const float*)d.dx + ((size_t)b * d.Nt + s) * d.lddx;
+            float v[NK];
+#pragma unroll
+            for (int k = 0; k < NK; ++k) {
+                const int c = lane + 64 * k;
+                v[k] = c < D ? g[c] : 0.f;
+            }
+            if (m == -2) {
+                if (d.d_reg_tokens) {
+                    float* rrow = (float*)d.d_reg_tokens + (size_t)s * D;
+#pragma unroll
+                    for (int k = 0; k < NK; ++k)
+                        if (lane + 64 * k < D) unsafeAtomicAdd(rrow + lane + 64 * k, v[k]);
+                }
+                continue;
+            }
+            const fm_embed_bwd_mod& md = d.mods[m];
+            const int src = __builtin_amdgcn_readlane(l_src, i);
+            const int posrow = __builtin_amdgcn_readlane(l_pos, i);
+            const bool to_mask_token = d.is_decoder && md.kind == FM_KIND_TOK;
+            if (m != cur) {
+                flush();
+                cur = m; cur_mask = to_mask_token;
+#pragma unroll
+                for (int k = 0; k < NK; ++k) racc[k] = 0.f;
+                if (lane == 0) { used[m] = 1; if (to_mask_token) used[d.n_mods] = 1; }
+            }
+            float* trow = nullptr;
+            if (to_mask_token) {}
+            else if ((md.kind == FM_KIND_TOK || md.kind == FM_KIND_SEQ) && md.d_table && !(md.has_padding_idx && src == md.padding_idx))
+                trow = (float*)md.d_table + (size_t)src * D;
+            else if (md.kind == FM_KIND_SEQ_EMB && md.d_proj_bias) trow = (float*)md.d_proj_bias;
+            float* prow = md.d_pos ? (float*)md.d_pos + (size_t)posrow * D : nullptr;
+#pragma unroll
+            for (int k = 0; k < NK; ++k) racc[k] += v[k];
             if (trow) {
-                unsafeAtomicAdd(trow + c * 4, v.x); unsafeAtomicAdd(trow + c * 4 + 1, v.y);
-                unsafeAtomicAdd(trow + c * 4 + 2, v.z); unsafeAtomicAdd(trow + c * 4 + 3, v.w);
+#pragma unroll
+                for (int k = 0; k < NK; ++k)
+                    if (lane + 64 * k < D) unsafeAtomicAdd(trow + lane + 64 * k, v[k]);
             }
             if (prow) {
-                unsafeAtomicAdd(prow + c * 4, v.x); unsafeAtomicAdd(prow + c * 4 + 1, v.y);
-                unsafeAtomicAdd(prow + c * 4 + 2, v.z); unsafeAtomicAdd(prow + c * 4 + 3, v.w);
+#pragma unroll
+                for (int k = 0; k < NK; ++k)
+                    if (lane + 64 * k < D) unsafeAtomicAdd(prow + lane + 64 * k, v[k]);
             }
         }
     }
@@ -323,10 +338,10 @@
     __syncthreads();
     for (int m = 0; m < d.n_mods; ++m) {
         if (!used[m] || !d.mods[m].d_mod_emb) continue;
-        for (int c = threadIdx.x; c < D; c += 256) unsafeAtomicAdd((float*)d.mods[m].d_mod_emb + c, acc[(size_t)m * D + c]);
+        for (int c = threadIdx.x; c < D; c += blockDim.x) unsafeAtomicAdd((float*)d.mods[m].d_mod_emb + c, acc[(size_t)m * D + c]);
     }
     if (used[d.n_mods] && d.d_mask_token)
-        for (int c = threadIdx.x; c < D; c += 256) unsafeAtomicAdd((float*)d.d_mask_token + c, acc[(size_t)d.n_mods * D + c]);
+        for (int c = threadIdx.x; c < D; c += blockDim.x) unsafeAtomicAdd((float*)d.d_mask_token + c, acc[(size_t)d.n_mods * D + c]);
 }
 
 __global__ void dense_decoder_mask_kernel(const int32_t* cs, const int16_t* mod, uint8_t* out, int B, int M, int causal, int use_cs, int use_sep) {
@@ -382,10 +397,21 @@
     FM_CHECK_ARG(d->n_mods > 0 && d->n_mods <= FM_MAX_MODS && d->dim % 4 == 0 && d->dim <= 2048 && d->lddx % 4 == 0, "fm_embed_bwd: bad shape (dim <= 2048)");
     const size_t lds = (size_t)(d->n_mods + 1) * d->dim * sizeof(float);
     FM_CHECK_ARG(lds <= 150 * 1024, "fm_embed_bwd: %zu bytes of LDS needed", lds);
-    static bool once = (hipFuncSetAttribute((const void*)embed_bwd_kernel, hipFuncAttributeMaxDynamicSharedMemorySize, 150 * 1024) == hipSuccess);
-    (void)once;
+    static const int spw_env = [] { const char* e = getenv("FOURM_EMBED_BWD_SPW"); return e ? atoi(e) : 4; }();
+    const int spw = spw_env >= 4 ? 4 : spw_env >= 2 ? 2 : 1;
     const int slices = d->batch >= 2048 ? 1 : d->batch >= 1024 ? 2 : 4;
-    hipLaunchKernelGGL(embed_bwd_kernel, dim3(d->batch, slices), dim3(256), lds, (hipStream_t)stream, *d);
+    const dim3 grid((d->batch + spw - 1) / spw, slices);
+#define LAUNCH_EMBED_BWD(NK)                                                                                                                   \
+    {                                                                                                                                          \
+        static bool once = (hipFuncSetAttribute((const void*)embed_bwd_kernel<NK>, hipFuncAttributeMaxDynamicSharedMemorySize, 150 * 1024) == hipSuccess); \
+        (void)once;                                                                                                                            \
+        hipLaunchKernelGGL(embed_bwd_kernel<NK>, grid, dim3(256 * spw), lds, (hipStream_t)stream, *d);                                         \
+    }
+    if (d->dim <= 256) LAUNCH_EMBED_BWD(4)
+    else if (d->dim <= 768) LAUNCH_EMBED_BWD(12)
+    else if (d->dim <= 1024) LAUNCH_EMBED_BWD(16)
+    else LAUNCH_EMBED_BWD(32)
+#undef LAUNCH_EMBED_BWD
     FM_CHECK_LAUNCH("fm_embed_bwd");
     return 0;
 }
diff --git a/ml-4m_amd/fourm/hip/_lib.py b/ml-4m_amd/fourm/hip/_lib.py
--- a/ml-4m_amd/fourm/hip/_lib.py
+++ b/ml-4m_amd/fourm/hip/_lib.py
@@ -138,6 +138,10 @@
                 ("n_mods", i32), ("batch", i32), ("dim", i32), ("Nt", i32), ("lddx", i32), ("is_decoder", i32)]
 
 
+class LnReduceJob(C.Structure):
+    _fields_ = [("partial", vp), ("dst", vp), ("n_partial", i32), ("D", i32)]
+
+
 class EmaJob(C.Structure):
     _fields_ = [("ema", vp), ("model", vp), ("n", i64), ("first_chunk", i64)]
 
@@ -157,6 +161,9 @@
 layernorm_fwd_res = _sig("fm_layernorm_fwd_res", vp, i32, vp, i32, vp, i32, vp, vp, vp, i32, i32, vp, vp, vp, i32, i32, f32, vp)
 layernorm_bwd = _sig("fm_layernorm_bwd", vp, i32, vp, vp, i32, vp, vp, vp, vp, vp, i32, vp, i32, vp, vp, i32, i32, vp)
 layernorm_bwd_h = _sig("fm_layernorm_bwd_h", vp, i32, vp, i32, vp, i32, vp, vp, vp, vp, vp, i32, vp, i32, vp, i32, i32, vp)
+layernorm_bwd_partial_rows = _sig("fm_layernorm_bwd_partial_rows", i32)
+layernorm_bwd_partial = _sig("fm_layernorm_bwd_partial", vp, i32, vp, vp, i32, vp, i32, vp, vp, vp, vp, vp, i32, vp, i32, vp, vp, i32, i32, i32, vp)
+ln_reduce_partials = _sig("fm_ln_reduce_partials", P(LnReduceJob), C.c_int, vp)
 attn_fwd = _sig("fm_attn_fwd", P(AttnArgs), vp)
 attn_bwd = _sig("fm_attn_bwd", P(AttnArgs), vp)
 attn_decode = _sig("fm_attn_decode", P(AttnDecodeArgs), vp)
@@ -283,7 +290,7 @@
 token_usage = _sig("fm_token_usage", vp, i32, i64, i64, i32, vp, vp, vp)
 EXPORTS = ["fm_reconst_loss_scratch", "fm_reconst_loss", "fm_scale_f32", "fm_mask_out_samples", "fm_ema_update", "fm_diffusion_pair", "fm_token_usage", "fm_lpips_stem", "fm_lpips_stem_bwd", "fm_maxpool2x2_nhwc", "fm_lpips_distance", "fm_lpips_tap_bwd", "fm_feat_distance", "fm_quick_gelu_bwd", "fm_quick_gelu_bwd_f32", "fm_clip_embed_ln_bwd", "fm_tap_add", "fm_clip_embed_ln", "fm_attn_decode", "fm_vit_patch_rows", "fm_vit_emb_rows", "fm_vit_colsum", "fm_lora_apply", "fm_lora_grad", "fm_vq_assign_wide", "fm_memcodes_assign", "fm_convnext_block", "fm_split3_bf16", "fm_unet_im2col", "fm_groupnorm_nhwc", "fm_add_bf16", "fm_silu_f32_to_bf16", "fm_timestep_embedding", "fm_unet_attention", "fm_diffusion_x0", "fm_quantile_abs",
            "fm_diffusion_step", "fm_unpack_image_u8", "fm_unpack_ids_u16", "fm_unpack_mask_bits", "fm_decoder_attention_from_target", "fm_guidance_combine", "fm_image_mask", "fm_token_budgets", "fm_span_mask", "fm_vq_code_stats", "fm_vq_ema_update", "fm_vq_code_bias", "fm_vq_assign_bias", "fm_vq_code_stats_raw", "fm_vq_ema_update_euclid", "fm_vq_unpatchify", "fm_vq_latent_grad", "fm_tanh_bwd_f32", "fm_embed_rows_f32", "fm_vq_patchify_ex", "fm_vq_cls_emb_bwd", "fm_vq_latent_grad_normalized", "fm_abi_version", "fm_last_error", "fm_gemm_nt", "fm_set_gemm_nt_config", "fm_get_gemm_nt_config", "fm_set_reserved_cus", "fm_get_reserved_cus", "fm_bf16_to_f32_scaled", "fm_add_bf16_f32", "fm_scale_rows_bf16", "fm_gemm_tn", "fm_gemm_tn_multi", "fm_set_gemm_tn_config", "fm_get_gemm_tn_config", "fm_set_tn_transpose_read",
-           "fm_get_tn_transpose_read", "fm_layernorm_fwd", "fm_layernorm_fwd_res", "fm_layernorm_bwd", "fm_layernorm_bwd_h", "fm_headnorm_fwd", "fm_headnorm_bwd", "fm_attn_fwd", "fm_attn_bwd",
+           "fm_get_tn_transpose_read", "fm_layernorm_fwd", "fm_layernorm_fwd_res", "fm_layernorm_bwd", "fm_layernorm_bwd_h", "fm_layernorm_bwd_partial_rows", "fm_layernorm_bwd_partial", "fm_ln_reduce_partials", "fm_headnorm_fwd", "fm_headnorm_bwd", "fm_attn_fwd", "fm_attn_bwd",
            "fm_set_attn_transpose_read", "fm_get_attn_transpose_read", "fm_select_embed", "fm_embed_bwd",
            "fm_dense_decoder_mask", "fm_segment_rows", "fm_gather_rows", "fm_cross_entropy", "fm_swiglu_bwd",
            "fm_gelu_bwd", "fm_cast_pad", "fm_transpose_cast_pad", "fm_shadow_refresh", "fm_fold_colscale_grad", "fm_colsum", "fm_f32_to_bf16", "fm_adamw", "fm_adamw_shadow",
diff --git a/ml-4m_amd/fourm/hip/engine.py b/ml-4m_amd/fourm/hip/engine.py
--- a/ml-4m_amd/fourm/hip/engine.py
+++ b/ml-4m_amd/fourm/hip/engine.py
@@ -17,6 +17,7 @@
 DEFER_RESIDUAL = os.environ.get("FOURM_DEFER_RESIDUAL", "1") == "1"
 HOIST_CTX = os.environ.get("FOURM_HOIST_CTX", "1") == "1"
 LN_BWD_FROM_H = os.environ.get("FOURM_LN_BWD_FROM_H", "1") == "1"
+LN_BWD_PARTIAL = os.environ.get("FOURM_LN_BWD_PARTIAL", "1") == "1"
 DP_RESERVE_ALWAYS = os.environ.get("FOURM_DP_RESERVE_ALWAYS", "0") == "1"
 
 
@@ -129,6 +130,7 @@
 
 
 class FourMEngine:
+    _ln_jobs = None
     _pending = None
     _drop_now = None
     drop_uniforms = None
@@ -249,6 +251,7 @@
 
     def _stage(self, name):
         if self.reducer is not None:
+            self._ln_flush()
             self.reducer.stage_done(name)
 
     def grad_view(self, p):
@@ -821,8 +824,24 @@
     def _ln_bwd(self, norm, dy, x, sv, key, g, g_bf, R, dres, dy_row_map=None):
         dw = self._g(norm.weight)
         db = self._g(norm.bias) if isinstance(norm.bias, nn.Parameter) else None
+        jobs = self._ln_jobs
+        if jobs is not None and dw is not None and dy.dtype != torch.float32:
+            P, D = ops.layernorm_bwd_partial_rows(R), norm.weight.numel()
+            pw = self.ws.get(f"bwd.lnp{len(jobs)}", (P, D), torch.float32)
+            pb = self.ws.get(f"bwd.lnp{len(jobs) + 1}", (P, D), torch.float32) if db is not None else None
+            ops.layernorm_bwd_partial(dy, x, norm.weight, sv[key + ".mu"], sv[key + ".rs"], g, pw, pb=pb, dres=dres, dx_bf16=g_bf,
+                                      dy_row_map=dy_row_map, R=R, h=sv.get(key + ".h"))
+            jobs.append((pw, P, dw))
+            if pb is not None:
+                jobs.append((pb, P, db))
+            return
         ops.layernorm_bwd(dy, x, norm.weight, sv[key + ".mu"], sv[key + ".rs"], g, dres=dres, dx_bf16=g_bf, dw=dw, db=db,
                           dy_row_map=dy_row_map, R=R, h=sv.get(key + ".h"))
+
+    def _ln_flush(self):
+        if self._ln_jobs:
+            ops.ln_reduce_partials(self._ln_jobs)
+            self._ln_jobs = []
 
     def _mlp_bwd(self, mlp, sv, g_bf, R, Rp):
         bf, D, Hp, Hd = self.adt, self.D, self.Hp, self.Hd
@@ -992,6 +1011,13 @@
         if c is None:
             raise RuntimeError("train_backward without a preceding training forward")
         self._ctx, self._dw_jobs = None, None
+        self._ln_jobs = [] if LN_BWD_PARTIAL else None
+        try:
+            self._train_backward(c, grad_scale)
+        finally:
+            self._ln_jobs = None
+
+    def _train_backward(self, c, grad_scale):
         if self.reducer is not None:
             self.reducer.begin()
             if getattr(self.reducer, "reserved_cus", 0):
@@ -1076,6 +1102,7 @@
             elif e.kind == L.KIND_SEQ_EMB and e.emb_proj.weight.requires_grad:
                 ops.gemm_tn(ge_bf, enc["seqemb_rows"], self.grad_view(e.emb_proj.weight), N=D, K=e.emb_proj.weight.shape[1], R=Rc)
         self._embed_bwd(enc, ge, dctx, False)
+        self._ln_flush()
         if self.reducer is not None:
             self.reducer.finish()
             if getattr(self.reducer, "reserved_cus", 0) and not DP_RESERVE_ALWAYS:
diff --git a/ml-4m_amd/fourm/hip/ops.py b/ml-4m_amd/fourm/hip/ops.py
--- a/ml-4m_amd/fourm/hip/ops.py
+++ b/ml-4m_amd/fourm/hip/ops.py
@@ -288,6 +288,30 @@
         return _ln_bwd(dy, x, w, mean, rstd, dx, dres, dx_bf16, dw, db, dy_row_map, R)
 
 
+def layernorm_bwd_partial_rows(R):
+    return int(L.layernorm_bwd_partial_rows(R))
+
+
+def layernorm_bwd_partial(dy, x, w, mean, rstd, dx, pw, *, pb=None, dres=None, dx_bf16=None, dy_row_map=None, R=None, h=None):
+    R = x.shape[0] if R is None else R
+    D = w.numel()
+    use_h = h is not None and pb is None and dy_row_map is None
+    with _prof("layernorm_bwd", 0.0, R * D * (2 + (2 if use_h else 4) + 4 + 4 + (2 if dx_bf16 is not None else 0))):
+        L.check(L.layernorm_bwd_partial(_p(dy), _ld(dy), _p(dy_row_map), _p(h) if use_h else None, _ld(h) if use_h else 0, _p(x), _ld(x), _p(w),
+                                        _p(mean), _p(rstd), _p(dres), _p(dx), _ld(dx), _p(dx_bf16), _ld(dx_bf16) if dx_bf16 is not None else 0,
+                                        _p(pw), _p(pb), pw.shape[0], R, D, _stream()))
+    return layernorm_bwd_partial_rows(R)
+
+
+def ln_reduce_partials(jobs):
+    arr = (L.LnReduceJob * len(jobs))()
+    for i, (part, n, dst) in enumerate(jobs):
+        assert part.dtype == torch.float32 and dst.dtype == torch.float32 and part.is_contiguous() and part.shape[0] >= n and part.shape[1] == dst.numel()
+        arr[i].partial, arr[i].dst, arr[i].n_partial, arr[i].D = _p(part), _p(dst), n, dst.numel()
+    with _prof("layernorm_bwd", 0.0, sum(4.0 * n * dst.numel() for _, n, dst in jobs)):
+        L.check(L.ln_reduce_partials(arr, len(jobs), _stream()))
+
+
 def _ln_bwd(dy, x, w, mean, rstd, dx, dres, dx_bf16, dw, db, dy_row_map, R):
     if dy.dtype == torch.float32:
         L.check(L.layernorm_bwd_f32(_p(dy), _ld(dy), _p(dy_row_map), _p(x), _ld(x), _p(w), _p(mean), _p(rstd), _p(dres), _p(dx), _ld(dx),
```

After: 1.185 million tokens/s (median of 6 runs). About the same (+0.6%).
